# meyer-lab/cmtf-pls

Hardware: AMD Instinct MI355X
Metric: nipals_iters_per_sec (higher is better)
Workload: dtype f32

## Files before the change

### cmtf_pls_amd/_lib.py

```python
from __future__ import annotations

import ctypes
import os
from ctypes import c_char_p, c_double, c_int, c_int64, c_size_t, c_uint64, c_void_p

_HERE = os.path.dirname(os.path.abspath(__file__))
LIB_PATH = os.environ.get("CMTFPLS_LIB") or os.path.join(_HERE, "lib", "libcmtfpls.so")

_P = c_void_p

class XcovBlock(ctypes.Structure):
    _fields_ = [("S", _P), ("S2", _P), ("colcnt", _P), ("n_samples", c_double), ("order", c_int), ("A", c_int), ("B", c_int),
                ("n_squarings", c_int), ("Z", _P), ("wA", _P), ("wB", _P), ("info", _P)]


class KfoldState(ctypes.Structure):
    _fields_ = [("I", c_int), ("A", c_int), ("B", c_int), ("M", c_int), ("K", c_int), ("R", c_int)] + [
        (name, _P) for name in ("fold_of", "S", "mean", "Yk", "Gy", "WA", "WB", "Q", "Wa", "Wb", "T", "Gt", "coef", "Rm", "tm",
                                "Tout", "vec", "n_iter", "status", "part")]


SIGNATURES = {
    "cmtfpls_xcov_iterate_blocks_f64": (c_int, [ctypes.POINTER(XcovBlock), c_int, c_int, _P, _P, _P, _P, _P, c_int, _P, c_size_t, _P]),
    "cmtfpls_abi_version": (c_int, []),
    "cmtfpls_last_error": (c_char_p, []),
    "cmtfpls_clear_error": (c_int, []),
    "cmtfpls_status_to_host": (c_int, [_P, _P, c_size_t, _P, _P]),
    "cmtfpls_colstats_workspace_bytes": (c_size_t, [c_int64, c_int64]),
    "cmtfpls_colstats_f32": (c_int, [_P, c_int64, c_int64, _P, _P, _P, c_size_t, _P]),
    "cmtfpls_colstats_f64": (c_int, [_P, c_int64, c_int64, _P, _P, _P, c_size_t, _P]),
    "cmtfpls_sweep_partials": (c_int, []),
    "cmtfpls_center_f32": (c_int, [_P, c_int64, c_int64, _P, _P, _P, _P]),
    "cmtfpls_center_f64": (c_int, [_P, c_int64, c_int64, _P, _P, _P, _P]),
    "cmtfpls_mode0_contract_workspace_bytes": (c_size_t, [c_int64, c_int64]),
    "cmtfpls_mode0_contract_f32": (c_int, [_P, c_int64, c_int64, _P, _P, c_int, _P, c_size_t, _P]),
    "cmtfpls_mode0_contract_f64": (c_int, [_P, c_int64, c_int64, _P, _P, c_int, _P, c_size_t, _P]),
    "cmtfpls_mode0_contract_yq_f32": (c_int, [_P, c_int64, c_int64, _P, c_int, c_int, _P, _P, c_int, _P, c_size_t, _P]),
    "cmtfpls_mode0_contract_yq_f64": (c_int, [_P, c_int64, c_int64, _P, c_int, c_int, _P, _P, c_int, _P, c_size_t, _P]),
    "cmtfpls_colscale_f64": (c_int, [_P, c_int64, _P, c_double, _P]),
    "cmtfpls_rank1_workspace_bytes": (c_size_t, [c_int, c_int]),
    "cmtfpls_rank1_score_f64": (c_int, [_P, c_int, c_int, _P, _P, _P, c_int, _P, c_int, _P, _P, c_size_t, _P]),
    "cmtfpls_rank1_f64": (c_int, [_P, c_int, c_int, _P, _P, _P, _P, c_int, _P, c_size_t, _P]),
    "cmtfpls_rank1_launches_f64": (c_int, [_P, c_int, c_int, _P, _P, _P, _P, c_int, _P, c_size_t, _P]),
    "cmtfpls_rank1_chain_enable": (None, [c_int]),
    "cmtfpls_rank1_chain_enabled": (c_int, []),
    "cmtfpls_normalize_f64": (c_int, [_P, c_int64, _P, _P]),
    "cmtfpls_rank1_tensor_workspace_bytes": (c_size_t, [_P, c_int]),
    "cmtfpls_rank1_tensor_f64": (c_int, [_P, _P, c_int, c_double, _P, c_int, _P, c_int, _P, c_size_t, _P]),
    "cmtfpls_kron_f64": (c_int, [_P, c_int, _P, c_int, _P, _P]),
    "cmtfpls_xcov_workspace_bytes": (c_size_t, [c_int64, c_int64, c_int]),
    "cmtfpls_xcov_f32": (c_int, [_P, c_int64, c_int64, _P, c_int, c_int, _P, c_int, _P, c_size_t, _P]),
    "cmtfpls_xcov_f64": (c_int, [_P, c_int64, c_int64, _P, c_int, c_int, _P, c_int, _P, c_size_t, _P]),
    "cmtfpls_quadform_f64": (c_int, [_P, c_int, _P, _P, _P, _P]),
    "cmtfpls_xcov_iterate_f64": (c_int, [_P, c_int, c_int, c_int, _P, _P, _P, _P, _P, c_int, _P, _P, _P, c_int, _P, c_size_t, _P, c_size_t, _P]),
    "cmtfpls_s_downdate_f64": (c_int, [_P, c_int, c_int, c_int, _P, _P, _P, _P, _P, _P]),
    "cmtfpls_project_rows_f32": (c_int, [_P, c_int64, c_int, c_int, c_int, _P, _P, _P, _P, c_int, _P]),
    "cmtfpls_project_rows_f64": (c_int, [_P, c_int64, c_int, c_int, c_int, _P, _P, _P, _P, c_int, _P]),
    "cmtfpls_project_rows2_f32": (c_int, [_P, c_int, c_int, _P, _P, _P, _P, c_int, c_int, _P, _P, _P, c_int64, c_int, _P, c_int, _P]),
    "cmtfpls_project_rows2_f64": (c_int, [_P, c_int, c_int, _P, _P, _P, _P, c_int, c_int, _P, _P, _P, c_int64, c_int, _P, c_int, _P]),
    "cmtfpls_project_rows_idx_f32": (c_int, [_P, _P, c_int64, c_int, c_int, c_int, _P, _P, _P, _P, c_int, _P]),
    "cmtfpls_project_rows_idx_f64": (c_int, [_P, _P, c_int64, c_int, c_int, c_int, _P, _P, _P, _P, c_int, _P]),
    "cmtfpls_project_rows2_idx_f32": (c_int, [_P, c_int, c_int, _P, _P, _P, _P, c_int, c_int, _P, _P, _P, _P, c_int64, c_int, _P, c_int, _P]),
    "cmtfpls_project_rows2_idx_f64": (c_int, [_P, c_int, c_int, _P, _P, _P, _P, c_int, c_int, _P, _P, _P, _P, c_int64, c_int, _P, c_int, _P]),
    "cmtfpls_allreduce_sum_f64": (c_int, [_P, _P, c_size_t, _P]),
    "cmtfpls_allreduce_sum_f32": (c_int, [_P, _P, c_size_t, _P]),
    "cmtfpls_axpy_scalar_f64": (c_int, [_P, c_int64, _P, _P, _P]),
    "cmtfpls_xcov_deflate_f32": (c_int, [_P, c_int64, c_int, c_int, _P, c_int, c_int, _P, _P, _P, _P, _P, _P, c_size_t, _P]),
    "cmtfpls_xcov_deflate_f64": (c_int, [_P, c_int64, c_int, c_int, _P, c_int, c_int, _P, _P, _P, _P, _P, _P, c_size_t, _P]),
    "cmtfpls_xcov_stats_workspace_bytes": (c_size_t, [c_int64, c_int64, c_int]),
    "cmtfpls_xcov_stats_f32": (c_int, [_P, c_int64, c_int64, _P, c_int, c_int, _P, _P, _P, c_size_t, _P]),
    "cmtfpls_xcov_stats_f64": (c_int, [_P, c_int64, c_int64, _P, c_int, c_int, _P, _P, _P, c_size_t, _P]),
    "cmtfpls_xcov_ssq_workspace_bytes": (c_size_t, [c_int64, c_int64, c_int]),
    "cmtfpls_xcov_ssq_f32": (c_int, [_P, c_int64, c_int64, _P, c_int, c_int, _P, _P, _P, _P, c_size_t, _P]),
    "cmtfpls_xcov_ssq_f64": (c_int, [_P, c_int64, c_int64, _P, c_int, c_int, _P, _P, _P, _P, c_size_t, _P]),
    "cmtfpls_score_contract_workspace_bytes": (c_size_t, [c_int64, c_int64]),
    "cmtfpls_score_contract_f32": (c_int, [_P, c_int64, c_int, c_int, _P, _P, _P, _P, _P, c_double, _P, _P, _P, _P, c_size_t, _P]),
    "cmtfpls_score_contract_f64": (c_int, [_P, c_int64, c_int, c_int, _P, _P, _P, _P, _P, c_double, _P, _P, _P, _P, c_size_t, _P]),
    "cmtfpls_kr_axpy_f64": (c_int, [_P, c_int, c_int, _P, _P, c_int, c_int, _P, _P]),
    "cmtfpls_xcov_f32_mixed": (c_int, [_P, c_int64, c_int64, _P, c_int, c_int, _P, c_int, _P, c_size_t, _P]),
    "cmtfpls_mttkrp_f32_mixed": (c_int, [_P, c_int64, c_int, c_int, _P, _P, c_int, _P, c_int, _P]),
    "cmtfpls_mttkrp_f32": (c_int, [_P, c_int64, c_int, c_int, _P, _P, c_int, _P, c_int, _P]),
    "cmtfpls_mttkrp_f64": (c_int, [_P, c_int64, c_int, c_int, _P, _P, c_int, _P, c_int, _P]),
    "cmtfpls_score_f32": (c_int, [_P, c_int64, c_int, c_int, _P, _P, _P, _P, _P]),
    "cmtfpls_score_f64": (c_int, [_P, c_int64, c_int, c_int, _P, _P, _P, _P, _P]),
    "cmtfpls_score_s_f64": (c_int, [_P, c_int, c_int, c_int, _P, _P, _P, _P]),
    "cmtfpls_deflate_contract_workspace_bytes": (c_size_t, [c_int64, c_int64]),
    "cmtfpls_deflate_contract_yq_f32": (c_int, [_P, c_int64, c_int, c_int, _P, _P, _P, _P, c_int, c_int, _P, _P, c_int, _P, _P, c_size_t, _P]),
    "cmtfpls_deflate_contract_yq_f64": (c_int, [_P, c_int64, c_int, c_int, _P, _P, _P, _P, c_int, c_int, _P, _P, c_int, _P, _P, c_size_t, _P]),
    "cmtfpls_score_gram_f32": (c_int, [_P, c_int64, c_int, c_int, _P, _P, _P, _P, _P, c_int, c_int, _P, _P]),
    "cmtfpls_score_gram_f64": (c_int, [_P, c_int64, c_int, c_int, _P, _P, _P, _P, _P, c_int, c_int, _P, _P]),
    "cmtfpls_q_update_f64": (c_int, [_P, c_int, c_int, _P, c_int, _P, _P, _P, _P]),
    "cmtfpls_deflate_f32": (c_int, [_P, c_int64, c_int, c_int, _P, _P, _P, _P, _P]),
    "cmtfpls_deflate_f64": (c_int, [_P, c_int64, c_int, c_int, _P, _P, _P, _P, _P]),
    "cmtfpls_score_deflate_f32": (c_int, [_P, c_int64, c_int, c_int, _P, _P, _P, _P, _P, _P]),
    "cmtfpls_score_deflate_f64": (c_int, [_P, c_int64, c_int, c_int, _P, _P, _P, _P, _P, _P]),
    "cmtfpls_small_workspace_bytes": (c_size_t, []),
    "cmtfpls_gram_tn_f64": (c_int, [_P, c_int, c_int, _P, c_int, c_int, c_int64, _P, _P, c_size_t, _P]),
    "cmtfpls_rowdot_f64": (c_int, [_P, c_int, c_int, c_int64, _P, _P, _P, _P, _P, c_size_t, _P]),
    "cmtfpls_scores_mean_f64": (c_int, [_P, c_int, c_int64, _P, _P]),
    "cmtfpls_y_deflate_f64": (c_int, [_P, c_int, c_int, c_int64, _P, c_int, c_int, _P, _P, _P, _P, c_size_t, _P]),
    "cmtfpls_sum_f64": (c_int, [_P, c_int64, _P, _P]),
    "cmtfpls_normal_solve_f64": (c_int, [_P, _P, c_int, _P, c_int, _P]),
    "cmtfpls_normal_solve_workspace_bytes": (c_size_t, [c_int]),
    "cmtfpls_normal_solve_ws_f64": (c_int, [_P, _P, c_int, _P, c_int, _P, c_size_t, _P]),
    "cmtfpls_unit_upper_solve_rows_f64": (c_int, [_P, c_int64, c_int, c_int, _P, _P, _P, _P]),
    "cmtfpls_kr_gram_row_f64": (c_int, [_P, c_int, c_int, c_int, _P, c_int, _P]),
    "cmtfpls_kr_gram_f64": (c_int, [_P, c_int, c_int, _P, c_int, c_double, _P]),
    "cmtfpls_khatri_rao_f64": (c_int, [_P, c_int, _P, c_int, c_int, _P, _P]),
    "cmtfpls_predict_rows_f64": (c_int, [_P, c_int64, c_int, c_int, _P, c_int, _P, _P, c_int, _P]),
    "cmtfpls_recon_f32": (c_int, [_P, c_int64, c_int, c_int, _P, _P, c_int, c_int, _P, _P, _P]),
    "cmtfpls_recon_f64": (c_int, [_P, c_int64, c_int, c_int, _P, _P, c_int, c_int, _P, _P, _P]),
    "cmtfpls_recon_r2_workspace_bytes": (c_size_t, [c_int64, c_int64]),
    "cmtfpls_recon_r2_f32": (c_int, [_P, _P, c_int64, c_int, c_int, _P, _P, c_int, c_int, _P, _P, _P, c_size_t, _P]),
    "cmtfpls_recon_r2_f64": (c_int, [_P, _P, c_int64, c_int, c_int, _P, _P, c_int, c_int, _P, _P, _P, c_size_t, _P]),
    "cmtfpls_loo_fold_workspace_bytes": (c_size_t, [c_int, c_int, c_int, c_int, c_int]),
    "cmtfpls_loo_tpls_f64": (c_int, [_P, _P, _P, _P, c_int, c_int, c_int, c_int, c_int, c_double, c_int, c_int, c_int, _P, _P, _P, c_size_t, _P]),
    "cmtfpls_loo_xcov_fold_workspace_bytes": (c_size_t, [c_int, c_int, c_int, c_int, c_int]),
    "cmtfpls_kfold_xcov_workspace_bytes": (c_size_t, [c_int64, c_int64, c_int, c_int]),
    "cmtfpls_kfold_xcov_f32": (c_int, [_P, c_int64, c_int, c_int, _P, c_int, _P, _P, c_int, _P, _P, _P, _P, _P, c_size_t, _P]),
    "cmtfpls_kfold_xcov_f64": (c_int, [_P, c_int64, c_int, c_int, _P, c_int, _P, _P, c_int, _P, _P, _P, _P, _P, c_size_t, _P]),
    "cmtfpls_kfold_row_tiles": (c_int, [c_int64]),
    "cmtfpls_kfold_part_stride": (c_int, []),
    "cmtfpls_kfold_inner_workspace_bytes": (c_size_t, [c_int, c_int, c_int]),
    "cmtfpls_kfold_inner_f64": (c_int, [ctypes.POINTER(KfoldState), c_int, c_double, c_int, _P, c_size_t, _P]),
    "cmtfpls_kfold_epilogue_f64": (c_int, [ctypes.POINTER(KfoldState), c_int, c_int, _P, _P]),
    "cmtfpls_kfold_inner_coupled_workspace_bytes": (c_size_t, [ctypes.POINTER(KfoldState), c_int]),
    "cmtfpls_kfold_inner_coupled_f64": (c_int, [ctypes.POINTER(KfoldState), c_int, c_int, c_double, c_int, _P, c_size_t, _P]),
    "cmtfpls_kfold_combine_scores_f64": (c_int, [_P, c_int, c_int64, _P, _P]),
    "cmtfpls_kfold_wide_xcov_workspace_bytes": (c_size_t, [c_int64, c_int64, c_int, c_int]),
    "cmtfpls_kfold_wide_xcov_f32": (c_int, [_P, c_int64, c_int, c_int, _P, c_int, _P, _P, c_int, _P, _P, _P, _P, _P, c_size_t, _P]),
    "cmtfpls_kfold_wide_xcov_f64": (c_int, [_P, c_int64, c_int, c_int, _P, c_int, _P, _P, c_int, _P, _P, _P, _P, _P, c_size_t, _P]),
    "cmtfpls_kfold_inner_grouped_f64": (c_int, [ctypes.POINTER(KfoldState), _P, c_int, c_int, c_double, c_int, _P, c_size_t, _P]),
    "cmtfpls_kfold_epilogue_grouped_f64": (c_int, [ctypes.POINTER(KfoldState), _P, c_int, c_int, c_int, _P, _P]),
    "cmtfpls_kfold_epilogue_splits_f64": (c_int, [ctypes.POINTER(KfoldState), c_int, c_int, c_int, _P, _P]),
    "cmtfpls_loo_xcov_f64": (c_int, [_P, _P, _P, _P, c_int, c_int, c_int, c_int, c_int, c_double, c_int, c_int, c_int, _P, _P, _P, c_size_t, _P]),
    "cmtfpls_fit_small_workspace_bytes": (c_size_t, [c_int, c_int, c_int, c_int]),
    "cmtfpls_fit_small_f64": (c_int, [_P, _P, c_int, c_int, c_int, c_int, c_int, c_double, c_int] + [_P] * 11 + [_P, c_size_t, _P]),
    "cmtfpls_add_noise_f32": (c_int, [_P, c_int64, c_double, c_uint64, c_uint64, c_double, _P]),
    "cmtfpls_add_noise_f64": (c_int, [_P, c_int64, c_double, c_uint64, c_uint64, c_double, _P]),
    "cmtfpls_ceiling_max_blocks": (c_int, []),
    "cmtfpls_ceiling_read": (c_int, [_P, c_size_t, c_int64, c_int, _P, c_int, _P]),
    "cmtfpls_ceiling_rmw": (c_int, [_P, c_size_t, c_int64, c_int, c_int, _P]),
    "cmtfpls_ceiling_copy": (c_int, [_P, _P, c_size_t, c_int64, c_int, c_int, _P]),
}

_lib = None


class CmtfplsError(RuntimeError):
    pass


def load():
    global _lib
    if _lib is not None:
        return _lib
    if not os.path.exists(LIB_PATH):
        raise CmtfplsError(
            f"{LIB_PATH} not found: build the HIP extension first (python -c 'import __graft_entry__ as g; g.build()'). "
            "cmtf_pls_amd has no CPU fallback."
        )
    lib = ctypes.CDLL(LIB_PATH)
    for name, (res, args) in SIGNATURES.items():
        fn = getattr(lib, name)
        fn.restype = res
        fn.argtypes = args
    _lib = lib
    return lib


def check(rc: int, what: str = "") -> None:
    if rc != 0:
        msg = load().cmtfpls_last_error()
        raise CmtfplsError(f"{what or 'cmtfpls call'} failed with status {rc}: {msg.decode() if msg else ''}")
```

### cmtf_pls_amd/backend.py

```python
from __future__ import annotations

import ctypes
from typing import Optional, Tuple

import torch

from . import _lib

_SUFFIX = {torch.float32: "f32", torch.float64: "f64"}


def _ptr(t: Optional[torch.Tensor]):
    return None if t is None else t.data_ptr()


class HipBackend:
    name = "hip"

    def __init__(self, device: Optional[torch.device] = None):
        self.lib = _lib.load()
        if not torch.cuda.is_available():
            raise _lib.CmtfplsError("cmtf_pls_amd needs a ROCm GPU (torch.cuda.is_available() is False); there is no CPU fallback")
        self.device = torch.device(device) if device is not None else torch.device("cuda", torch.cuda.current_device())
        self.n_partials = int(self.lib.cmtfpls_sweep_partials())
        self._ws = {}
        self._status_slots = {}
        self.rank1_squarings = 30
        self.rank1_chain_side = 256 if self.lib.cmtfpls_rank1_chain_enabled() else 0

    def _stream(self):
        return torch.cuda.current_stream(self.device).cuda_stream

    def _workspace(self, key: str, nbytes: int) -> torch.Tensor:
        buf = self._ws.get(key)
        if buf is None or buf.numel() < nbytes:
            buf = torch.empty(max(int(nbytes), 256), dtype=torch.uint8, device=self.device)
            self._ws[key] = buf
        return buf

    def clear_error(self) -> bool:
        return bool(self.lib.cmtfpls_clear_error())

    def empty(self, *shape, dtype=torch.float64) -> torch.Tensor:
        return torch.empty(*shape, dtype=dtype, device=self.device)

    def zeros(self, *shape, dtype=torch.float64) -> torch.Tensor:
        return torch.zeros(*shape, dtype=dtype, device=self.device)

    def _fn(self, base: str, X: torch.Tensor):
        if X.dtype not in _SUFFIX:
            raise TypeError(f"X must be float32 or float64 on device, got {X.dtype}")
        assert X.is_contiguous() and X.device == self.device
        return getattr(self.lib, f"cmtfpls_{base}_{_SUFFIX[X.dtype]}")

    def _close_partials(self, part: torch.Tensor) -> torch.Tensor:
        out = self.empty(1)
        _lib.check(self.lib.cmtfpls_sum_f64(_ptr(part), part.numel(), _ptr(out), self._stream()), "sum")
        return out

    def ceiling(self, op: str, buf: torch.Tensor, row_bytes: int = 0, blocks: int = 2048,
                dst: Optional[torch.Tensor] = None, map: int = 0) -> bool:
        nbytes = buf.numel() * buf.element_size()
        if op == "read":
            sink = self._workspace("ceiling_sink", 4 * self.lib.cmtfpls_ceiling_max_blocks())
            rc = self.lib.cmtfpls_ceiling_read(_ptr(buf), nbytes, int(row_bytes), int(map), _ptr(sink), int(blocks), self._stream())
        elif op == "rmw":
            rc = self.lib.cmtfpls_ceiling_rmw(_ptr(buf), nbytes, int(row_bytes), int(map), int(blocks), self._stream())
        elif op == "copy":
            assert dst is not None and dst.numel() * dst.element_size() >= nbytes
            rc = self.lib.cmtfpls_ceiling_copy(_ptr(buf), _ptr(dst), nbytes, int(row_bytes), int(map), int(blocks), self._stream())
        else:
            raise ValueError(op)
        if rc == 4:
            return False
        _lib.check(rc, "ceiling_" + op)
        return True

    def colstats(self, X2: torch.Tensor) -> Tuple[torch.Tensor, torch.Tensor]:
        I, P = X2.shape
        ws = self._workspace("contract", self.lib.cmtfpls_colstats_workspace_bytes(I, P))
        colsum, colcnt = self.empty(P), self.empty(P)
        _lib.check(self._fn("colstats", X2)(_ptr(X2), I, P, _ptr(colsum), _ptr(colcnt), _ptr(ws), ws.numel(), self._stream()), "colstats")
        return colsum, colcnt

    def center(self, X2: torch.Tensor, mean: torch.Tensor, want_rowcnt: bool) -> Tuple[Optional[torch.Tensor], torch.Tensor]:
        I, P = X2.shape
        rowcnt = self.empty(I) if want_rowcnt else None
        part = self.empty(self.n_partials)
        _lib.check(self._fn("center", X2)(_ptr(X2), I, P, _ptr(mean), _ptr(rowcnt), _ptr(part), self._stream()), "center")
        return rowcnt, self._close_partials(part)

    def mode0_contract(self, X2: torch.Tensor, u: torch.Tensor, masked: bool, out: Optional[torch.Tensor] = None) -> torch.Tensor:
        I, P = X2.shape
        ws = self._workspace("contract", self.lib.cmtfpls_mode0_contract_workspace_bytes(I, P))
        Z = out if out is not None else self.empty(P)
        _lib.check(self._fn("mode0_contract", X2)(_ptr(X2), I, P, _ptr(u), _ptr(Z), int(masked), _ptr(ws), ws.numel(), self._stream()), "mode0_contract")
        return Z

    def mode0_contract_yq(self, X2: torch.Tensor, Y: torch.Tensor, q: torch.Tensor, masked: bool,
                          out: torch.Tensor) -> Optional[torch.Tensor]:
        I, P = X2.shape
        ws = self._workspace("contract", self.lib.cmtfpls_mode0_contract_workspace_bytes(I, P))
        rc = self._fn("mode0_contract_yq", X2)(_ptr(X2), I, P, _ptr(Y), Y.stride(0), Y.shape[1], _ptr(q), _ptr(out), int(masked),
                                               _ptr(ws), ws.numel(), self._stream())
        if rc == 4:
            return None
        _lib.check(rc, "mode0_contract_yq")
        return out

    def colscale(self, Z: torch.Tensor, colcnt: torch.Tensor, n_samples: float) -> None:
        _lib.check(self.lib.cmtfpls_colscale_f64(_ptr(Z), Z.numel(), _ptr(colcnt), float(n_samples), self._stream()), "colscale")

    def rank1(self, Z: torch.Tensor, A: int, B: int, wA: torch.Tensor, wB: torch.Tensor,
              info: Optional[torch.Tensor] = None, n_squarings: Optional[int] = None, launches: bool = False) -> None:
        ws = self._workspace("rank1", self.lib.cmtfpls_rank1_workspace_bytes(A, B))
        fn = self.lib.cmtfpls_rank1_launches_f64 if launches else self.lib.cmtfpls_rank1_f64
        _lib.check(fn(_ptr(Z), A, B, _ptr(wA), _ptr(wB), None, _ptr(info), int(n_squarings or self.rank1_squarings),
                      _ptr(ws), ws.numel(), self._stream()), "rank1")

    def rank1_chain_gave_up(self) -> None:
        self.lib.cmtfpls_rank1_chain_enable(0)
        self.rank1_chain_side = 0

    def rank1_tensor(self, Z: torch.Tensor, dims, tol: float, factors: torch.Tensor,
                     info: Optional[torch.Tensor] = None, n_squarings: Optional[int] = None) -> None:
        import ctypes
        arr = (ctypes.c_int * len(dims))(*[int(d) for d in dims])
        ws = self._workspace("rank1t", self.lib.cmtfpls_rank1_tensor_workspace_bytes(arr, len(dims)))
        _lib.check(self.lib.cmtfpls_rank1_tensor_f64(_ptr(Z), arr, len(dims), float(tol), _ptr(factors), factors.stride(0), _ptr(info),
                                                     int(n_squarings or self.rank1_squarings), _ptr(ws), ws.numel(), self._stream()),
                   "rank1_tensor")

    def kron(self, a: torch.Tensor, b: torch.Tensor, out: torch.Tensor) -> torch.Tensor:
        _lib.check(self.lib.cmtfpls_kron_f64(_ptr(a), a.numel(), _ptr(b), b.numel(), _ptr(out), self._stream()), "kron")
        return out

    def normalize(self, v: torch.Tensor) -> None:
        _lib.check(self.lib.cmtfpls_normalize_f64(_ptr(v), v.numel(), None, self._stream()), "normalize")

    def xcov(self, X2: torch.Tensor, Y: torch.Tensor, masked: bool, out: Optional[torch.Tensor] = None,
             mixed: bool = False) -> Optional[torch.Tensor]:
        I, P = X2.shape
        M = Y.shape[1]
        ws = self._workspace("contract", self.lib.cmtfpls_xcov_workspace_bytes(I, P, M))
        S = out if out is not None else self.empty(M, P)
        fn = self.lib.cmtfpls_xcov_f32_mixed if (mixed and X2.dtype == torch.float32) else self._fn("xcov", X2)
        _lib.check(fn(_ptr(X2), I, P, _ptr(Y), Y.stride(0), M, _ptr(S), int(masked), _ptr(ws), ws.numel(), self._stream()), "xcov")
        return S

    def xcov_deflate(self, X2: torch.Tensor, A: int, B: int, Y: torch.Tensor, t: torch.Tensor, wA: torch.Tensor, wB: torch.Tensor,
                     out: torch.Tensor) -> Optional[torch.Tensor]:
        I, P = X2.shape
        M = Y.shape[1]
        if M > 64 or P % 4 != 0 or P != A * B:
            return None
        ws = self._workspace("contract", self.lib.cmtfpls_xcov_ssq_workspace_bytes(I, P, M))
        ssq = self.empty(1)
        rc = self._fn("xcov_deflate", X2)(_ptr(X2), I, A, B, _ptr(Y), Y.stride(0), M, _ptr(t), _ptr(wA), _ptr(wB), _ptr(out), _ptr(ssq),
                                          _ptr(ws), ws.numel(), self._stream())
        if rc == 4:
            return None
        _lib.check(rc, "xcov_deflate")
        return ssq

    def rank1_score(self, Z: torch.Tensor, A: int, B: int, wA: torch.Tensor, wB: torch.Tensor, S: torch.Tensor, tq: torch.Tensor,
                    info: Optional[torch.Tensor] = None, n_squarings: Optional[int] = None) -> torch.Tensor:
        M = S.shape[0]
        assert S.is_contiguous() and S.shape[1] == A * B and tq.numel() >= M
        ws = self._workspace("rank1", self.lib.cmtfpls_rank1_workspace_bytes(A, B))
        _lib.check(self.lib.cmtfpls_rank1_score_f64(_ptr(Z), A, B, _ptr(wA), _ptr(wB), _ptr(info),
                                                    int(n_squarings if n_squarings is not None else self.rank1_squarings),
                                                    _ptr(S), M, _ptr(tq), _ptr(ws), ws.numel(), self._stream()), "rank1_score")
        return tq

    def xcov_ssq(self, X2: torch.Tensor, Y: torch.Tensor, mean: torch.Tensor, out: torch.Tensor):
        I, P = X2.shape
        M = Y.shape[1]
        ws = self._workspace("contract", self.lib.cmtfpls_xcov_ssq_workspace_bytes(I, P, M))
        ssq = self.empty(1)
        assert mean.is_contiguous() and mean.numel() == P and mean.dtype == torch.float64
        _lib.check(self._fn("xcov_ssq", X2)(_ptr(X2), I, P, _ptr(Y), Y.stride(0), M, _ptr(out), _ptr(mean), _ptr(ssq), _ptr(ws), ws.numel(),
                                            self._stream()), "xcov_ssq")
        return out, ssq

    def xcov_stats(self, X2: torch.Tensor, Y: torch.Tensor, out: torch.Tensor):
        I, P = X2.shape
        M = Y.shape[1]
        if M > 64 or not X2.is_contiguous():
            return None
        ws = self._workspace("contract", self.lib.cmtfpls_xcov_stats_workspace_bytes(I, P, M))
        stats = self.empty(2 * P)
        rc = self._fn("xcov_stats", X2)(_ptr(X2), I, P, _ptr(Y), Y.stride(0), M, _ptr(out), _ptr(stats), _ptr(ws), ws.numel(), self._stream())
        if rc == 4:
            return None
        _lib.check(rc, "xcov_stats")
        return out, stats

    def status_snapshot(self, status: torch.Tensor, slot: int, slots: Optional[dict] = None):
        slots = self._status_slots if slots is None else slots
        ent = slots.get((slot, status.numel()))
        if ent is None:
            host, ev = torch.empty(status.numel(), dtype=torch.float64, pin_memory=True), torch.cuda.Event()
            ev.record(torch.cuda.current_stream(self.device))
            ent = slots[(slot, status.numel())] = (host, ev, host.numpy(), host.data_ptr(), ev.cuda_event, status.numel() * 8)
        rc = self.lib.cmtfpls_status_to_host(status.data_ptr(), ent[3], ent[5], ent[4], self._stream())
        if rc:
            _lib.check(rc, "status_to_host")
        return ent

    def status_wait(self, token) -> "np.ndarray":
        token[1].synchronize()
        return token[2]

    def xcov_iterate_plan(self, S: torch.Tensor, A: int, B: int, q_cur: torch.Tensor, Z: torch.Tensor, wA: torch.Tensor,
                          wB: torch.Tensor, status: torch.Tensor, q_new: torch.Tensor, G: torch.Tensor):
        M, P = S.shape
        wc = self._workspace("contract", self.lib.cmtfpls_mode0_contract_workspace_bytes(M, P))
        wr = self._workspace("rank1", self.lib.cmtfpls_rank1_workspace_bytes(A, B))
        keep = (S, q_cur, Z, wA, wB, status, q_new, G, wc, wr)
        fn = self.lib.cmtfpls_xcov_iterate_f64
        head = (_ptr(S), M, A, B, _ptr(q_cur), _ptr(Z), _ptr(wA), _ptr(wB), status[1:3].data_ptr())
        tail = (_ptr(wc), wc.numel(), _ptr(wr), wr.numel())
        qn, Gp, du2 = _ptr(q_new), _ptr(G), status[0:1].data_ptr()
        stream = self._stream

        def enqueue(n_squarings: int, first: bool, _keep=keep) -> None:
            rc = fn(*head, n_squarings, qn, Gp, du2, 1 if first else 0, *tail, stream())
            if rc:
                _lib.check(rc, "xcov_iterate")
        return enqueue

    def xcov_iterate(self, S: torch.Tensor, A: int, B: int, q_cur: torch.Tensor, Z: torch.Tensor, wA: torch.Tensor,
                     wB: torch.Tensor, info: torch.Tensor, n_squarings: int, q_new: torch.Tensor, G: torch.Tensor,
                     du2: torch.Tensor, first: bool) -> None:
        M, P = S.shape
        wc = self._workspace("contract", self.lib.cmtfpls_mode0_contract_workspace_bytes(M, P))
        wr = self._workspace("rank1", self.lib.cmtfpls_rank1_workspace_bytes(A, B))
        _lib.check(self.lib.cmtfpls_xcov_iterate_f64(_ptr(S), M, A, B, _ptr(q_cur), _ptr(Z), _ptr(wA), _ptr(wB), _ptr(info),
                                                     int(n_squarings), _ptr(q_new), _ptr(G), _ptr(du2), int(first),
                                                     _ptr(wc), wc.numel(), _ptr(wr), wr.numel(), self._stream()), "xcov_iterate")

    def xcov_blocks_plan(self, blocks, M: int, q_cur: torch.Tensor, tq: torch.Tensor, q_new: torch.Tensor, G: torch.Tensor,
                         status: torch.Tensor):
        nb = len(blocks)
        if M > 64 or any(b["order"] not in (2, 3) for b in blocks) or tq.numel() != nb * M or not tq.is_contiguous():
            return None
        arr = (_lib.XcovBlock * nb)()
        need = 256
        for i, b in enumerate(blocks):
            for name in ("S", "S2", "colcnt", "Z", "wA", "wB"):
                t = b.get(name)
                assert t is None or (t.is_contiguous() and t.dtype == torch.float64 and t.device == self.device), name
                setattr(arr[i], name, _ptr(t))
            arr[i].n_samples, arr[i].order, arr[i].A, arr[i].B = float(b["n_samples"]), int(b["order"]), int(b["A"]), int(b["B"])
            arr[i].info = status[1 + 2 * i: 3 + 2 * i].data_ptr()
            if b["order"] == 3:
                need = max(need, self.lib.cmtfpls_rank1_workspace_bytes(b["A"], b["B"]))
        wr = self._workspace("rank1", need)
        keep = (blocks, q_cur, tq, q_new, G, status, wr, arr)
        fn, stream = self.lib.cmtfpls_xcov_iterate_blocks_f64, self._stream
        args = (nb, M, _ptr(q_cur), _ptr(tq), _ptr(q_new), _ptr(G), status[0:1].data_ptr())
        tail = (_ptr(wr), wr.numel())

        def enqueue(n_squarings, first: bool, _keep=keep) -> None:
            for i in range(nb):
                arr[i].n_squarings = int(n_squarings[i])
            rc = fn(arr, *args, 1 if first else 0, *tail, stream())
            if rc:
                _lib.check(rc, "xcov_iterate_blocks")
        return enqueue

    def s_downdate(self, S: torch.Tensor, A: int, B: int, ya: torch.Tensor, wA: torch.Tensor, wB: torch.Tensor,
                   q: torch.Tensor, v: torch.Tensor) -> None:
        assert S.is_contiguous() and S.shape[1] == A * B
        _lib.check(self.lib.cmtfpls_s_downdate_f64(_ptr(S), S.shape[0], A, B, _ptr(ya), _ptr(wA), _ptr(wB), _ptr(q), _ptr(v),
                                                   self._stream()), "s_downdate")

    def kr_axpy(self, v: torch.Tensor, A: int, B: int, WA: torch.Tensor, WB: torch.Tensor, k: int, coef: torch.Tensor) -> torch.Tensor:
        assert WA.is_contiguous() and WB.is_contiguous() and WA.shape[1] == WB.shape[1] and coef.numel() >= k
        _lib.check(self.lib.cmtfpls_kr_axpy_f64(_ptr(v), A, B, _ptr(WA), _ptr(WB), WA.shape[1], int(k), _ptr(coef), self._stream()), "kr_axpy")
        return v

    def axpy_scalar(self, y: torch.Tensor, a: torch.Tensor, x: Optional[torch.Tensor] = None) -> torch.Tensor:
        assert y.is_contiguous() and y.dtype == torch.float64 and a.numel() >= 1 and (x is None or (x.is_contiguous() and x.numel() == y.numel()))
        _lib.check(self.lib.cmtfpls_axpy_scalar_f64(_ptr(y), y.numel(), _ptr(a), _ptr(x), self._stream()), "axpy_scalar")
        return y

    def total(self, v: torch.Tensor) -> torch.Tensor:
        assert v.is_contiguous() and v.dtype == torch.float64
        return self._close_partials(v)

    def quadform(self, G: torch.Tensor, q: torch.Tensor, q_old: torch.Tensor, out: torch.Tensor) -> torch.Tensor:
        _lib.check(self.lib.cmtfpls_quadform_f64(_ptr(G), G.shape[0], _ptr(q), _ptr(q_old), _ptr(out), self._stream()), "quadform")
        return out

    def mttkrp(self, X2: torch.Tensor, A: int, B: int, WA: torch.Tensor, WB: torch.Tensor, out: torch.Tensor,
               mixed: bool = False) -> Optional[torch.Tensor]:
        R = WA.shape[1]
        assert WA.is_contiguous() and WB.is_contiguous() and out.stride(1) == 1
        fn = self.lib.cmtfpls_mttkrp_f32_mixed if (mixed and X2.dtype == torch.float32) else self._fn("mttkrp", X2)
        rc = fn(_ptr(X2), X2.shape[0], A, B, _ptr(WA), _ptr(WB), R, _ptr(out), out.stride(0), self._stream())
        if rc == 4:
            return None
        _lib.check(rc, "mttkrp")
        return out

    def score(self, X2, A, B, wA, wB, rowcnt, out) -> torch.Tensor:
        _lib.check(self._fn("score", X2)(_ptr(X2), X2.shape[0], A, B, _ptr(wA), _ptr(wB), _ptr(rowcnt), _ptr(out), self._stream()), "score")
        return out

    def score_s(self, S, A, B, wA, wB, out) -> torch.Tensor:
        assert S.dtype == torch.float64 and S.is_contiguous()
        _lib.check(self.lib.cmtfpls_score_s_f64(_ptr(S), S.shape[0], A, B, _ptr(wA), _ptr(wB), _ptr(out), self._stream()), "score_s")
        return out

    def score_contract(self, X2, A, B, wA, wB, shift, t, Z, sub_own=None, add_other=None, alpha: float = 1.0,
                       csum: Optional[torch.Tensor] = None) -> Optional[torch.Tensor]:
        I, P = X2.shape
        if not X2.is_contiguous() or P != A * B:
            return None
        for v in (sub_own, add_other):
            assert v is None or (v.is_contiguous() and v.numel() == I and v.dtype == torch.float64)
        nbytes = self.lib.cmtfpls_score_contract_workspace_bytes(I, P)
        ws = self._workspace("score_contract", max(nbytes, 256))
        rc = self._fn("score_contract", X2)(_ptr(X2), I, A, B, _ptr(wA), _ptr(wB), _ptr(shift), _ptr(sub_own), _ptr(add_other), float(alpha),
                                            _ptr(t), _ptr(Z), _ptr(csum), _ptr(ws), ws.numel(), self._stream())
        if rc == 4:
            return None
        _lib.check(rc, "score_contract")
        return Z

    def score_gram(self, X2, A, B, wA, wB, rowcnt, out, Y: torch.Tensor, qpart: torch.Tensor) -> Optional[torch.Tensor]:
        assert qpart.numel() >= self.n_partials * Y.shape[1] and qpart.is_contiguous()
        rc = self._fn("score_gram", X2)(_ptr(X2), X2.shape[0], A, B, _ptr(wA), _ptr(wB), _ptr(rowcnt), _ptr(out),
                                        _ptr(Y), Y.stride(0), Y.shape[1], _ptr(qpart), self._stream())
        if rc == 4:
            return None
        _lib.check(rc, "score_gram")
        return out

    def q_update(self, q: torch.Tensor, qpart: Optional[torch.Tensor] = None, normalize: bool = True,
                 G: Optional[torch.Tensor] = None, q_prev: Optional[torch.Tensor] = None,
                 du2: Optional[torch.Tensor] = None, nparts: Optional[int] = None) -> None:
        M = q.numel()
        nrows = (nparts or self.n_partials) if qpart is not None else 0
        assert qpart is None or (qpart.is_contiguous() and qpart.numel() >= nrows * M)
        _lib.check(self.lib.cmtfpls_q_update_f64(_ptr(qpart), nrows, M, _ptr(q), int(normalize),
                                                 _ptr(G), _ptr(q_prev), _ptr(du2), self._stream()), "q_update")

    def deflate(self, X2, A, B, t, wA, wB) -> torch.Tensor:
        part = self.empty(self.n_partials)
        _lib.check(self._fn("deflate", X2)(_ptr(X2), X2.shape[0], A, B, _ptr(t), _ptr(wA), _ptr(wB), _ptr(part), self._stream()), "deflate")
        return self._close_partials(part)

    def deflate_contract_yq(self, X2, A, B, t, wA, wB, Y: torch.Tensor, q: torch.Tensor, masked: bool,
                            out: torch.Tensor) -> Optional[torch.Tensor]:
        I, P = X2.shape
        ws = self._workspace("deflate_contract", self.lib.cmtfpls_deflate_contract_workspace_bytes(I, P))
        ssq = self.empty(1)
        rc = self._fn("deflate_contract_yq", X2)(_ptr(X2), I, A, B, _ptr(t), _ptr(wA), _ptr(wB), _ptr(Y), Y.stride(0), Y.shape[1],
                                                 _ptr(q), _ptr(out), int(masked), _ptr(ssq), _ptr(ws), ws.numel(), self._stream())
        if rc == 4:
            return None
        _lib.check(rc, "deflate_contract_yq")
        return ssq

    def score_deflate(self, X2, A, B, wA, wB, rowcnt, out) -> Optional[torch.Tensor]:
        part = self.empty(self.n_partials)
        rc = self._fn("score_deflate", X2)(_ptr(X2), X2.shape[0], A, B, _ptr(wA), _ptr(wB), _ptr(rowcnt), _ptr(out), _ptr(part), self._stream())
        if rc == 4:
            return None
        _lib.check(rc, "score_deflate")
        return self._close_partials(part)

    def gram_tn(self, A: torch.Tensor, B: torch.Tensor, out: Optional[torch.Tensor] = None) -> torch.Tensor:
        if A.dim() == 1:
            A = A.unsqueeze(1)
        if B.dim() == 1:
            B = B.unsqueeze(1)
        assert A.stride(1) == 1 and B.stride(1) == 1 and A.shape[0] == B.shape[0]
        a, b = A.shape[1], B.shape[1]
        ws = self._workspace("small", self.lib.cmtfpls_small_workspace_bytes())
        C = out if out is not None else self.empty(a, b)
        assert C.numel() == a * b and C.is_contiguous()
        _lib.check(self.lib.cmtfpls_gram_tn_f64(_ptr(A), A.stride(0), a, _ptr(B), B.stride(0), b, A.shape[0], _ptr(C),
                                                _ptr(ws), ws.numel(), self._stream()), "gram_tn")
        return C

    def rowdot(self, Y: torch.Tensor, q: torch.Tensor, u_out: torch.Tensor, u_old: Optional[torch.Tensor],
               du2: Optional[torch.Tensor] = None) -> Optional[torch.Tensor]:
        ws = self._workspace("small", self.lib.cmtfpls_small_workspace_bytes())
        if u_old is not None and du2 is None:
            du2 = self.empty(1)
        _lib.check(self.lib.cmtfpls_rowdot_f64(_ptr(Y), Y.stride(0), Y.shape[1], Y.shape[0], _ptr(q), _ptr(u_out), _ptr(u_old),
                                               _ptr(du2) if u_old is not None else None,
                                               _ptr(ws), ws.numel(), self._stream()), "rowdot")
        return du2 if u_old is not None else None

    def normal_solve(self, G: torch.Tensor, g: torch.Tensor, out: Optional[torch.Tensor] = None) -> torch.Tensor:
        k = G.shape[0]
        assert G.is_contiguous() and G.shape == (k, k) and g.numel() == k
        b = out if out is not None else self.empty(k)
        if k <= 64:
            _lib.check(self.lib.cmtfpls_normal_solve_f64(_ptr(G), _ptr(g), k, _ptr(b), 1, self._stream()), "normal_solve")
        else:
            ws = self._workspace("normal_solve", self.lib.cmtfpls_normal_solve_workspace_bytes(k))
            _lib.check(self.lib.cmtfpls_normal_solve_ws_f64(_ptr(G), _ptr(g), k, _ptr(b), 1, _ptr(ws), ws.numel(), self._stream()),
                       "normal_solve")
        return b

    def unit_upper_solve_rows(self, M: torch.Tensor, U: torch.Tensor, shift: Optional[torch.Tensor] = None,
                              nan_flag: Optional[torch.Tensor] = None) -> torch.Tensor:
        I, R = M.shape
        assert M.stride(1) == 1 and U.is_contiguous() and U.shape == (R, R)
        assert shift is None or (shift.is_contiguous() and shift.numel() == R and shift.dtype == torch.float64)
        assert nan_flag is None or nan_flag.dtype == torch.int32
        _lib.check(self.lib.cmtfpls_unit_upper_solve_rows_f64(_ptr(M), I, M.stride(0), R, _ptr(U), _ptr(shift), _ptr(nan_flag),
                                                              self._stream()), "unit_upper_solve_rows")
        return M

    def kr_gram_row(self, L: torch.Tensor, a: int, g: torch.Tensor, first: bool) -> torch.Tensor:
        assert L.is_contiguous() and g.is_contiguous() and g.numel() >= a
        _lib.check(self.lib.cmtfpls_kr_gram_row_f64(_ptr(L), L.shape[0], L.shape[1], int(a), _ptr(g), int(first), self._stream()), "kr_gram_row")
        return g

    def kr_gram(self, L: torch.Tensor, G: torch.Tensor, first: bool) -> torch.Tensor:
        n, R = L.shape
        assert L.is_contiguous() and G.is_contiguous() and G.numel() == R * R
        _lib.check(self.lib.cmtfpls_kr_gram_f64(_ptr(L), n, R, _ptr(G), int(first), 1.0, self._stream()), "kr_gram")
        return G

    def khatri_rao(self, Am: torch.Tensor, Bm: torch.Tensor) -> torch.Tensor:
        na, R = Am.shape
        nb = Bm.shape[0]
        assert Am.is_contiguous() and Bm.is_contiguous() and Bm.shape[1] == R
        out = self.empty(na * nb, R)
        _lib.check(self.lib.cmtfpls_khatri_rao_f64(_ptr(Am), na, _ptr(Bm), nb, R, _ptr(out), self._stream()), "khatri_rao")
        return out

    def project_rows(self, X2: torch.Tensor, A: int, B: int, WA: torch.Tensor, WB: torch.Tensor, mean: Optional[torch.Tensor],
                     out: torch.Tensor, rows: Optional[torch.Tensor] = None) -> Optional[torch.Tensor]:
        I, R = X2.shape[0], WA.shape[1]
        assert WA.is_contiguous() and WB.is_contiguous() and out.stride(1) == 1 and out.shape == (I, R)
        if rows is not None:
            assert rows.dtype == torch.int64 and rows.is_contiguous() and rows.device == self.device
            rc = self._fn("project_rows_idx", X2)(_ptr(X2), _ptr(rows), rows.numel(), A, B, R, _ptr(WA), _ptr(WB), _ptr(mean), _ptr(out),
                                                  out.stride(0), self._stream())
        else:
            rc = self._fn("project_rows", X2)(_ptr(X2), I, A, B, R, _ptr(WA), _ptr(WB), _ptr(mean), _ptr(out), out.stride(0), self._stream())
        if rc == 4:
            return None
        _lib.check(rc, "project_rows")
        return out

    def project_rows2(self, X2s, As, Bs, WAs, WBs, means, out: torch.Tensor, rows: Optional[torch.Tensor] = None) -> Optional[torch.Tensor]:
        I, R = X2s[0].shape[0], WAs[0].shape[1]
        if X2s[0].dtype != X2s[1].dtype or X2s[1].shape[0] != I:
            return None
        assert all(w.is_contiguous() for w in list(WAs) + list(WBs)) and out.stride(1) == 1 and out.shape == (I, R)
        head = (_ptr(X2s[0]), As[0], Bs[0], _ptr(WAs[0]), _ptr(WBs[0]), _ptr(means[0]),
                _ptr(X2s[1]), As[1], Bs[1], _ptr(WAs[1]), _ptr(WBs[1]), _ptr(means[1]))
        if rows is not None:
            assert rows.dtype == torch.int64 and rows.is_contiguous() and rows.device == self.device
            rc = self._fn("project_rows2_idx", X2s[0])(*head, _ptr(rows), rows.numel(), R, _ptr(out), out.stride(0), self._stream())
        else:
            rc = self._fn("project_rows2", X2s[0])(*head, I, R, _ptr(out), out.stride(0), self._stream())
        if rc == 4:
            return None
        _lib.check(rc, "project_rows2")
        return out

    def predict_rows(self, S: torch.Tensor, Bm: torch.Tensor, mean: Optional[torch.Tensor]) -> Optional[torch.Tensor]:
        I, R = S.shape
        M = Bm.shape[1]
        assert S.stride(1) == 1 and Bm.is_contiguous() and Bm.shape[0] == R
        out = self.empty(I, M)
        rc = self.lib.cmtfpls_predict_rows_f64(_ptr(S), I, S.stride(0), R, _ptr(Bm), M, _ptr(mean), _ptr(out), M, self._stream())
        if rc == 4:
            return None
        _lib.check(rc, "predict_rows")
        return out

    def recon(self, T: torch.Tensor, WA: torch.Tensor, WB: torch.Tensor, mean: Optional[torch.Tensor], out: torch.Tensor) -> Optional[torch.Tensor]:
        I, R = T.shape
        A, B = WA.shape[0], WB.shape[0]
        assert T.stride(1) == 1 and WA.is_contiguous() and WB.is_contiguous() and out.is_contiguous() and out.numel() == I * A * B
        rc = self._fn("recon", out)(_ptr(T), I, T.stride(0), R, _ptr(WA), _ptr(WB), A, B, _ptr(mean), _ptr(out), self._stream())
        if rc == 4:
            return None
        _lib.check(rc, "recon")
        return out

    def recon_r2(self, X2: torch.Tensor, T: torch.Tensor, WA: torch.Tensor, WB: torch.Tensor, mean: Optional[torch.Tensor]) -> Optional[torch.Tensor]:
        I, P = X2.shape
        R = T.shape[1]
        A, B = WA.shape[0], WB.shape[0]
        assert X2.is_contiguous() and T.stride(1) == 1 and WA.is_contiguous() and WB.is_contiguous() and P == A * B
        ws = self._workspace("recon_r2", self.lib.cmtfpls_recon_r2_workspace_bytes(I, P))
        out = self.empty(2)
        rc = self._fn("recon_r2", X2)(_ptr(X2), _ptr(T), I, T.stride(0), R, _ptr(WA), _ptr(WB), A, B, _ptr(mean), _ptr(out),
                                     _ptr(ws), ws.numel(), self._stream())
        if rc == 4:
            return None
        _lib.check(rc, "recon_r2")
        return out

    def loo_tpls(self, X2: torch.Tensor, Y: torch.Tensor, A: int, B: int, R: int, tol: float, max_iter: int,
                 max_ws_bytes: Optional[int] = None, forms=("lds", "xcov")) -> Optional[Tuple[torch.Tensor, torch.Tensor, str]]:
        I, P = X2.shape
        M = Y.shape[1]
        assert X2.dtype == torch.float64 and Y.dtype == torch.float64 and X2.is_contiguous() and Y.is_contiguous() and P == A * B
        colsum_x, _ = self.colstats(X2)
        colsum_y, _ = self.colstats(Y)
        Ypred = self.empty(I, M)
        n_iter = torch.zeros(I, R, dtype=torch.int32, device=self.device)
        for form, per_fn, fn in (("lds", self.lib.cmtfpls_loo_fold_workspace_bytes, self.lib.cmtfpls_loo_tpls_f64),
                                 ("xcov", self.lib.cmtfpls_loo_xcov_fold_workspace_bytes, self.lib.cmtfpls_loo_xcov_f64)):
            if form not in forms:
                continue
            if fn(_ptr(X2), _ptr(Y), _ptr(colsum_x), _ptr(colsum_y), I, A, B, M, R, float(tol), int(max_iter), 0, 1, _ptr(Ypred),
                  _ptr(n_iter), None, 0, self._stream()) == 4:
                continue
            per = per_fn(I, A, B, M, R)
            budget = max_ws_bytes
            if budget is None:
                budget = (4 << 30) if form == "lds" else max(4 << 30, torch.cuda.mem_get_info(self.device)[0] // 3)
            chunk = max(1, min(I, int(budget // max(per, 1))))
            if form == "xcov":
                chunk = min(chunk, 512)
            declined = False
            ws = None
            for f0 in range(0, I, chunk):
                nf = min(chunk, I - f0)
                if ws is None:
                    ws = self._workspace("loo", per * min(chunk, I))
                rc = fn(_ptr(X2), _ptr(Y), _ptr(colsum_x), _ptr(colsum_y), I, A, B, M, R, float(tol), int(max_iter),
                        f0, nf, _ptr(Ypred), _ptr(n_iter), _ptr(ws), ws.numel(), self._stream())
                if rc == 4:
                    declined = True
                    break
                _lib.check(rc, "loo_" + form)
            if not declined:
                return Ypred, n_iter, form
        return None

    def kfold_xcov(self, X2: torch.Tensor, A: int, B: int, Y: torch.Tensor, order: torch.Tensor, fold_off: torch.Tensor, K: int,
                   ydev: torch.Tensor, S: torch.Tensor, mean: torch.Tensor) -> Optional[torch.Tensor]:
        I, P = X2.shape
        M = Y.shape[1]
        assert Y.dtype == torch.float64 and Y.is_contiguous() and order.dtype == torch.int32 and fold_off.dtype == torch.int32 and P == A * B
        ws = torch.empty(max(int(self.lib.cmtfpls_kfold_xcov_workspace_bytes(I, P, M, K)), 256), dtype=torch.uint8, device=self.device)
        stats = self.empty(2 * P)
        rc = self._fn("kfold_xcov", X2)(_ptr(X2), I, A, B, _ptr(Y), M, _ptr(order), _ptr(fold_off), K, _ptr(ydev), _ptr(S), _ptr(mean),
                                        _ptr(stats), _ptr(ws), ws.numel(), self._stream())
        if rc == 4:
            return None
        _lib.check(rc, "kfold_xcov")
        return stats

    def kfold_inner(self, state, a: int, tol: float, max_iter: int, ws: torch.Tensor) -> Optional[bool]:
        rc = self.lib.cmtfpls_kfold_inner_f64(ctypes.byref(state), int(a), float(tol), int(max_iter), _ptr(ws), ws.numel(), self._stream())
        if rc == 4:
            return None
        _lib.check(rc, "kfold_inner")
        return True

    def kfold_inner_workspace_bytes(self, A: int, B: int, K: int) -> int:
        return int(self.lib.cmtfpls_kfold_inner_workspace_bytes(A, B, K))

    def kfold_row_tiles(self, I: int) -> Tuple[int, int]:
        return int(self.lib.cmtfpls_kfold_row_tiles(I)), int(self.lib.cmtfpls_kfold_part_stride())

    def kfold_epilogue(self, state, stage: int, a: int, src: Optional[torch.Tensor]) -> Optional[bool]:
        rc = self.lib.cmtfpls_kfold_epilogue_f64(ctypes.byref(state), int(stage), int(a), _ptr(src), self._stream())
        if rc == 4:
            return None
        _lib.check(rc, "kfold_epilogue")
        return True

    def kfold_inner_coupled(self, views, a: int, tol: float, max_iter: int, ws: torch.Tensor) -> Optional[bool]:
        rc = self.lib.cmtfpls_kfold_inner_coupled_f64(views, len(views), int(a), float(tol), int(max_iter), _ptr(ws), ws.numel(),
                                                      self._stream())
        if rc == 4:
            return None
        _lib.check(rc, "kfold_inner_coupled")
        return True

    def kfold_inner_coupled_workspace_bytes(self, views) -> int:
        return int(self.lib.cmtfpls_kfold_inner_coupled_workspace_bytes(views, len(views)))

    def kfold_combine_scores(self, sc: torch.Tensor, out: torch.Tensor) -> torch.Tensor:
        assert sc.is_contiguous() and out.is_contiguous() and sc[0].numel() == out.numel()
        _lib.check(self.lib.cmtfpls_kfold_combine_scores_f64(_ptr(sc), sc.shape[0], out.numel(), _ptr(out), self._stream()),
                   "kfold_combine_scores")
        return out

    def kfold_wide_xcov(self, X2: torch.Tensor, A: int, B: int, Y: torch.Tensor, order: torch.Tensor, fold_off: torch.Tensor, K: int,
                        ydev: torch.Tensor, S: torch.Tensor, mean: torch.Tensor) -> Optional[torch.Tensor]:
        I, P = X2.shape
        W = Y.shape[1]
        assert Y.dtype == torch.float64 and Y.is_contiguous() and ydev.is_contiguous() and S.is_contiguous() and P == A * B
        assert order.dtype == torch.int32 and fold_off.dtype == torch.int32 and S.numel() == K * W * P and mean.numel() == K * P
        ws = torch.empty(max(int(self.lib.cmtfpls_kfold_wide_xcov_workspace_bytes(I, P, W, K)), 256), dtype=torch.uint8, device=self.device)
        stats = self.empty(2 * P)
        rc = self._fn("kfold_wide_xcov", X2)(_ptr(X2), I, A, B, _ptr(Y), W, _ptr(order), _ptr(fold_off), K, _ptr(ydev), _ptr(S),
                                             _ptr(mean), _ptr(stats), _ptr(ws), ws.numel(), self._stream())
        if rc == 4:
            return None
        _lib.check(rc, "kfold_wide_xcov")
        return stats

    def kfold_inner_grouped(self, state, model_fold: torch.Tensor, groups: int, a: int, tol: float, max_iter: int,
                            ws: torch.Tensor) -> Optional[bool]:
        assert model_fold.dtype == torch.int32 and model_fold.numel() == state.K
        rc = self.lib.cmtfpls_kfold_inner_grouped_f64(ctypes.byref(state), _ptr(model_fold), int(groups), int(a), float(tol), int(max_iter),
                                                      _ptr(ws), ws.numel(), self._stream())
        if rc == 4:
            return None
        _lib.check(rc, "kfold_inner_grouped")
        return True

    def kfold_epilogue_grouped(self, state, model_fold: torch.Tensor, groups: int, stage: int, a: int,
                               src: Optional[torch.Tensor]) -> Optional[bool]:
        assert model_fold.dtype == torch.int32 and model_fold.numel() == state.K
        rc = self.lib.cmtfpls_kfold_epilogue_grouped_f64(ctypes.byref(state), _ptr(model_fold), int(groups), int(stage), int(a), _ptr(src),
                                                         self._stream())
        if rc == 4:
            return None
        _lib.check(rc, "kfold_epilogue_grouped")
        return True

    def kfold_epilogue_splits(self, state, splits: int, stage: int, a: int, src: Optional[torch.Tensor]) -> Optional[bool]:
        rc = self.lib.cmtfpls_kfold_epilogue_splits_f64(ctypes.byref(state), int(splits), int(stage), int(a), _ptr(src), self._stream())
        if rc == 4:
            return None
        _lib.check(rc, "kfold_epilogue_splits")
        return True

    def fit_small(self, X2: torch.Tensor, Y: torch.Tensor, A: int, B: int, R: int, tol: float, max_iter: int):
        I, P = X2.shape
        M = Y.shape[1]
        if X2.dtype != torch.float64 or Y.dtype != torch.float64 or not (X2.is_contiguous() and Y.is_contiguous()) or I >= 2 ** 31 or P != A * B:
            return None
        nbytes = self.lib.cmtfpls_fit_small_workspace_bytes(I, A, B, M)
        T, U = self.empty(I, R), self.empty(I, R)
        WA, WB, Q = self.empty(A, R), self.empty(B, R), self.empty(M, R)
        small = self.empty(R * R + 2 * (R + 1))
        xm, ym = self.empty(P), self.empty(M)
        ints = torch.zeros(R + 1, dtype=torch.int32, device=self.device)
        ws = self._workspace("fit_small", max(nbytes, 256))
        rc = self.lib.cmtfpls_fit_small_f64(_ptr(X2), _ptr(Y), I, A, B, M, R, float(tol), int(max_iter), _ptr(T), _ptr(U), _ptr(WA), _ptr(WB),
                                            _ptr(Q), _ptr(small), small[R * R:].data_ptr(), _ptr(xm), _ptr(ym), _ptr(ints),
                                            ints[R:].data_ptr(), _ptr(ws), ws.numel(), self._stream())
        if rc == 4:
            return None
        _lib.check(rc, "fit_small")
        ih = ints.cpu().numpy()
        if ih[R] != 0:
            return None
        sh = small.cpu().numpy()
        return {"T": T, "U": U, "WA": WA, "WB": WB, "Q": Q, "x_mean": xm, "y_mean": ym, "coef": sh[:R * R].reshape(R, R).copy(),
                "ssq": sh[R * R:].reshape(R + 1, 2).copy(), "n_iter": [int(v) for v in ih[:R]]}

    def add_noise(self, X: torch.Tensor, sigma: float, seed: int, offset: int = 0, nan_fraction: float = 0.0) -> torch.Tensor:
        assert X.is_contiguous() and X.device == self.device
        _lib.check(self._fn("add_noise", X)(_ptr(X), X.numel(), float(sigma), int(seed) & (2 ** 64 - 1), int(offset), float(nan_fraction),
                                            self._stream()), "add_noise")
        return X

    def scores_mean(self, Ts: torch.Tensor, out: torch.Tensor) -> torch.Tensor:
        nb, I = Ts.shape
        _lib.check(self.lib.cmtfpls_scores_mean_f64(_ptr(Ts), nb, I, _ptr(out), self._stream()), "scores_mean")
        return out

    def y_deflate(self, Y: torch.Tensor, T: torch.Tensor, ncols: int, b: torch.Tensor, q: torch.Tensor) -> torch.Tensor:
        ws = self._workspace("small", self.lib.cmtfpls_small_workspace_bytes())
        ssq = self.empty(1)
        _lib.check(self.lib.cmtfpls_y_deflate_f64(_ptr(Y), Y.stride(0), Y.shape[1], Y.shape[0], _ptr(T), T.stride(0), ncols, _ptr(b), _ptr(q),
                                                  _ptr(ssq), _ptr(ws), ws.numel(), self._stream()), "y_deflate")
        return ssq
```

### cmtf_pls_amd/csrc/rank1.hip

```cpp
#include "common.hpp"
#include <atomic>

namespace cmtfpls {

constexpr int kTile = 16;
constexpr int kMaxTiles = 256;
constexpr int kMaxSteps = 48;

struct Rank1Ctl {
  int done;
  int final_buf;
  int steps_used;
  int last_step;
  double pad[6];
};
__host__ __device__ __forceinline__ size_t rank1_ctl_bytes(int nt) {
  return sizeof(Rank1Ctl) + ((size_t)(kMaxSteps + 2) * nt + 2 * (size_t)nt * nt) * sizeof(double);
}
__device__ __forceinline__ double* ctl_trace(Rank1Ctl* c, int nt, int step) { return reinterpret_cast<double*>(c + 1) + (size_t)step * nt; }
__device__ __forceinline__ double* ctl_fro(Rank1Ctl* c, int nt, int which) {
  return reinterpret_cast<double*>(c + 1) + (size_t)(kMaxSteps + 2) * nt + (size_t)which * nt * nt;
}

__device__ __forceinline__ double pow2_scale_from_trace(const double* parts, int nt, double* tr_out) {
  double tr = 0.0;
  for (int i = 0; i < nt; ++i) tr += parts[i];
  *tr_out = tr;
  if (!(tr > 0.0) || !isfinite(tr)) return 1.0;
  int e;
  frexp(tr, &e);
  return ldexp(1.0, -e);
}

typedef double d4r_t __attribute__((ext_vector_type(4)));

__global__ __launch_bounds__(kTile* kTile) void syrk_step_kernel(const double* __restrict__ M, int n, int k, int ld,
                                                                double* __restrict__ C, Rank1Ctl* __restrict__ ctl,
                                                                int step, int out_buf, double* __restrict__ C_keep) {
  __shared__ double red[4][kTile * kTile];
  __shared__ double diag[kTile];
  __shared__ double s_scale;
  __shared__ int s_done;
  __shared__ double fsum[4];
  __shared__ double tr_s[kMaxTiles];
  const int tx = threadIdx.x, ty = threadIdx.y, tid = ty * kTile + tx;
  const int lane = tid & 63, wv = tid >> 6, ri = lane & 15, kq = lane >> 4;
  const int nt = (n + kTile - 1) / kTile;
  const int i0 = blockIdx.y * kTile, j0 = blockIdx.x * kTile;

  constexpr int KC = 128, KW = 8;
  const bool ra = (i0 + ri) < n, rb = (j0 + ri) < n;
  const double* __restrict__ rowa = M + (int64_t)(ra ? i0 + ri : 0) * ld;
  const double* __restrict__ rowb = M + (int64_t)(rb ? j0 + ri : 0) * ld;
  const int cl = 32 * wv + KW * kq;
  double a[KW], b[KW];
#pragma unroll
  for (int s2 = 0; s2 < KW; ++s2) {
    const int c = cl + s2;
    const int cc = (c < k) ? c : 0;
    a[s2] = rowa[cc];
    b[s2] = rowb[cc];
  }

  double fro_in = 0.0;
  if (step >= 1) {
    int zero = 0;
    asm volatile("" : "+v"(zero));
    const int last_in = (&ctl->last_step)[zero];
    const int done_in = (&ctl->done)[zero] | ((last_in >= 0 && last_in < step) ? 1 : 0);
    const double* fp = ctl_fro(ctl, nt, (step - 1) & 1);
    const double trv = ctl_trace(ctl, nt, step - 1)[(tid < nt) ? tid : 0];
    double f = fp[(tid < nt * nt) ? tid : 0];
    if (tid < nt) tr_s[tid] = trv;
    if (tid >= nt * nt) f = 0.0;
    for (int i = tid + kTile * kTile; i < nt * nt; i += kTile * kTile) f += fp[i];
    f = wave_sum(f);
    if ((tid & 63) == 0) fsum[tid >> 6] = f;
    if (tid == 0) s_done = done_in;
    __syncthreads();
    fro_in = ((fsum[0] + fsum[1]) + fsum[2]) + fsum[3];
  }
  if (tid == 0) {
    int done = 0;
    double scale = 1.0;
    if (step == 0) {
      if (blockIdx.x == 0 && blockIdx.y == 0) { ctl->done = 0; ctl->final_buf = -1; ctl->steps_used = 0; ctl->last_step = -1; }
    } else {
      done = s_done;
      if (!done) {
        double tr1;
        scale = pow2_scale_from_trace(tr_s, nt, &tr1);
        const double rho = fro_in / (tr1 * tr1);
        const bool rank_one_in = !(tr1 > 0.0) || rho >= 1.0 - 1e-13;
        const bool rank_one_out = rho >= 1.0 - 1e-7;
        if (blockIdx.x == 0 && blockIdx.y == 0) {
          if (rank_one_in) { ctl->done = 1; ctl->final_buf = out_buf ^ 1; }
          else {
            ctl->steps_used = step;
            if (rank_one_out) { ctl->last_step = step; ctl->final_buf = out_buf; }
          }
        }
        if (rank_one_in) done = 1;
      }
    }
    s_scale = scale;
    s_done = done;
  }
  __syncthreads();
  if (s_done) return;
  const double scale = s_scale;

  d4r_t acc = d4r_t{0.0, 0.0, 0.0, 0.0};
  for (int kk = 0; kk < k; kk += KC) {
    if (kk > 0) {
#pragma unroll
      for (int s2 = 0; s2 < KW; ++s2) {
        const int c = kk + cl + s2;
        const int cc = (c < k) ? c : 0;
        a[s2] = rowa[cc];
        b[s2] = rowb[cc];
      }
    }
#pragma unroll
    for (int s2 = 0; s2 < KW; ++s2) {
      const bool cok = (kk + cl + s2) < k;
      const double av = (ra && cok) ? a[s2] : 0.0;
      const double bv = (rb && cok) ? b[s2] : 0.0;
      acc = __builtin_amdgcn_mfma_f64_16x16x4f64(av, bv, acc, 0, 0, 0);
    }
  }
#pragma unroll
  for (int e = 0; e < 4; ++e) red[wv][(kq + 4 * e) * kTile + ri] = acc[e];
  __syncthreads();
  double cacc = ((red[0][tid] + red[1][tid]) + red[2][tid]) + red[3][tid];
  cacc *= scale * scale;
  const bool inside = (i0 + ty < n && j0 + tx < n);
  if (inside) C[(int64_t)(i0 + ty) * n + (j0 + tx)] = cacc;
  if (inside && C_keep) C_keep[(int64_t)(i0 + ty) * n + (j0 + tx)] = cacc;
  {
    double sq = inside ? cacc * cacc : 0.0;
    sq = wave_sum(sq);
    if ((tid & 63) == 0) fsum[tid >> 6] = sq;
    __syncthreads();
    if (tid == 0) ctl_fro(ctl, nt, step & 1)[blockIdx.y * nt + blockIdx.x] = ((fsum[0] + fsum[1]) + fsum[2]) + fsum[3];
  }
  if (blockIdx.x == blockIdx.y) {
    if (tx == ty) diag[tx] = (i0 + ty < n) ? cacc : 0.0;
    __syncthreads();
    if (tid == 0) {
      double t = 0.0;
      for (int l = 0; l < kTile; ++l) t += diag[l];
      ctl_trace(ctl, nt, step)[blockIdx.x] = t;
    }
  }
}

constexpr unsigned long long kChainEmpty = ~0ull;
constexpr int kChainMaxSteps = 31;
constexpr int kChainSpin = 1 << 15;

__device__ __forceinline__ double chain_ld(const double* p) {
  return __longlong_as_double((long long)__hip_atomic_load(reinterpret_cast<const unsigned long long*>(p), __ATOMIC_RELAXED, __HIP_MEMORY_SCOPE_AGENT));
}
__device__ __forceinline__ void chain_st(double* p, double v) {
  unsigned long long b = (unsigned long long)__double_as_longlong(v);
  if (b == kChainEmpty) b = 0x7FF8000000000000ull;
  __hip_atomic_store(reinterpret_cast<unsigned long long*>(p), b, __ATOMIC_RELAXED, __HIP_MEMORY_SCOPE_AGENT);
}
__device__ __forceinline__ bool chain_empty(double v) { return (unsigned long long)__double_as_longlong(v) == kChainEmpty; }

__global__ __launch_bounds__(256) void chain_preset_kernel(unsigned long long* __restrict__ p, int64_t n) {
  for (int64_t i = (int64_t)blockIdx.x * 256 + threadIdx.x; i < n; i += (int64_t)gridDim.x * 256) p[i] = kChainEmpty;
}

#ifdef CMTFPLS_CHAIN_PROFILE
__device__ unsigned long long g_chain_prof[1024];
#define CHAIN_STAMP(slot) do { if (first_wg && tid == 0 && step < 32) g_chain_prof[step * 8 + (slot)] = __builtin_amdgcn_s_memrealtime(); } while (0)
#define CHAIN_COUNT(slot, v) do { if (first_wg && tid == 0 && step < 32) g_chain_prof[step * 8 + (slot)] = (unsigned long long)(v); } while (0)
#else
#define CHAIN_STAMP(slot) do { } while (0)
#define CHAIN_COUNT(slot, v) do { } while (0)
#endif

__global__ __launch_bounds__(kTile* kTile) void syrk_chain_kernel(const double* __restrict__ M0, int n, int k0,
                                                                 double* gbufs, double* trs, double* fros, double* gave_up,
                                                                 Rank1Ctl* __restrict__ ctl, int n_squarings) {
  constexpr int KC = 128, KW = 8, LDP = KC + 2;
  __shared__ __attribute__((aligned(16))) double pan[2][kTile][LDP];
  __shared__ double red[2][4][kTile * kTile];
  __shared__ double diag[2][kTile];
  __shared__ double fsum[2][4];
  __shared__ double cfro[2][4];
  __shared__ double ctr[2][kTile];
  __shared__ int cdead[2];
  const int tx = threadIdx.x, ty = threadIdx.y, tid = ty * kTile + tx;
  const int lane = tid & 63, wv = tid >> 6, ri = lane & 15, kq = lane >> 4;
  const int nt = (n + kTile - 1) / kTile, nt2 = nt * nt;
  const int i0 = blockIdx.y * kTile, j0 = blockIdx.x * kTile;
  const bool first_wg = blockIdx.x == 0 && blockIdx.y == 0;
  const bool ra = (i0 + ri) < n, rb = (j0 + ri) < n;
  const int cl = 32 * wv + KW * kq;
  const int64_t nn = (int64_t)n * n;
  const double qnan = __longlong_as_double(0x7FF8000000000000ll);
  bool dead = false;
  if (first_wg && tid == 0) { ctl->done = 0; ctl->final_buf = -1; ctl->steps_used = 0; ctl->last_step = -1; }
  if (tid < 2) cdead[tid] = 0;
  int last_step = -1;
  for (int step = 0; step <= n_squarings; ++step) {
    if (last_step >= 0) break;
    const int par = step & 1;
    const double* __restrict__ M = step == 0 ? M0 : gbufs + (int64_t)(step - 1) * nn;
    const int k = step == 0 ? k0 : n, ld = k;
    double* C = gbufs + (int64_t)step * nn;
    double a[KW], b[KW];
    double scale = 1.0;
    bool input_is_result = false;
    d4r_t acc = d4r_t{0.0, 0.0, 0.0, 0.0};
    CHAIN_STAMP(0);
    for (int kk = 0; kk < k; kk += KC) {
      if (step == 0) {
        const double* __restrict__ rowa = M + (int64_t)(ra ? i0 + ri : 0) * ld;
        const double* __restrict__ rowb = M + (int64_t)(rb ? j0 + ri : 0) * ld;
#pragma unroll
        for (int s2 = 0; s2 < KW; ++s2) {
          const int c = kk + cl + s2;
          const int cc = (c < k) ? c : 0;
          a[s2] = rowa[cc];
          b[s2] = rowb[cc];
        }
      } else {
        double va[8], vb[8], trv = 0.0, f = 0.0;
        const bool first_chunk = kk == 0;
        const double* tp = trs + (int64_t)(step - 1) * nt;
        const double* fp = fros + (int64_t)(step - 1) * nt2;
        unsigned offa[8], offb[8];
#pragma unroll
        for (int i = 0; i < 8; ++i) {
          const int e = tid + 256 * i, r = e >> 7, c = kk + (e & 127);
          const int cc = (c < k) ? c : 0;
          const int rra = (i0 + r < n) ? i0 + r : 0, rrb = (j0 + r < n) ? j0 + r : 0;
          offa[i] = (unsigned)(rra * ld + cc);
          offb[i] = (unsigned)(rrb * ld + cc);
        }
        int spins = 0;
        for (;;) {
          bool ok = true;
#pragma unroll
          for (int i = 0; i < 8; ++i) {
            va[i] = chain_ld(M + offa[i]);
            vb[i] = chain_ld(M + offb[i]);
          }
          if (first_chunk) {
            f = chain_ld(fp + ((tid < nt2) ? tid : 0));
            ok = !chain_empty(f);
            if (wv == 0) {
              trv = chain_ld(tp + ((lane < nt) ? lane : 0));
              ok = ok && !chain_empty(trv);
            }
          }
#pragma unroll
          for (int i = 0; i < 8; ++i) ok = ok && !chain_empty(va[i]) && !chain_empty(vb[i]);
          if (dead || __all(ok)) break;
          if (++spins > kChainSpin) {
            dead = true;
            if (lane == 0) chain_st(gave_up, 1.0);
            break;
          }
        }
        CHAIN_STAMP(1);
        CHAIN_COUNT(7, spins);
        if (kk > 0) __syncthreads();
#pragma unroll
        for (int i = 0; i < 8; ++i) {
          const int e = tid + 256 * i, r = e >> 7, c = e & 127;
          pan[0][r][c] = dead ? qnan : va[i];
          pan[1][r][c] = dead ? qnan : vb[i];
        }
        if (first_chunk) {
          const double fw = wave_sum((tid < nt2) ? f : 0.0);
          if (lane == 0) cfro[par][wv] = fw;
          if (wv == 0 && lane < nt) ctr[par][lane] = trv;
          if (dead && lane == 0) cdead[par] = 1;
        }
        __syncthreads();
        CHAIN_STAMP(2);
        if (first_chunk) {
          const double fro_in = ((cfro[par][0] + cfro[par][1]) + cfro[par][2]) + cfro[par][3];
          double tr1 = 0.0;
          for (int i = 0; i < nt; ++i) tr1 += ctr[par][i];
          if ((tr1 > 0.0) && isfinite(tr1)) {
            int e;
            frexp(tr1, &e);
            scale = ldexp(1.0, -e);
          }
          const bool gone = cdead[par] != 0;
          const double rho = fro_in / (tr1 * tr1);
          const bool rank_one_in = !gone && (!(tr1 > 0.0) || rho >= 1.0 - 1e-13);
          const bool rank_one_out = !gone && rho >= 1.0 - 1e-7;
          if (first_wg && tid == 0) {
            if (rank_one_in) { ctl->done = 1; ctl->final_buf = step - 1; }
            else {
              ctl->steps_used = step;
              if (rank_one_out) { ctl->last_step = step; ctl->final_buf = step; }
            }
          }
          if (rank_one_in) { input_is_result = true; break; }
          if (rank_one_out) last_step = step;
        }
#pragma unroll
        for (int s2 = 0; s2 < KW; ++s2) {
          a[s2] = pan[0][ri][cl + s2];
          b[s2] = pan[1][ri][cl + s2];
        }
      }
#pragma unroll
      for (int s2 = 0; s2 < KW; ++s2) {
        const bool cok = (kk + cl + s2) < k;
        const double av = (ra && cok) ? a[s2] : 0.0;
        const double bv = (rb && cok) ? b[s2] : 0.0;
        acc = __builtin_amdgcn_mfma_f64_16x16x4f64(av, bv, acc, 0, 0, 0);
      }
    }
    if (input_is_result) break;
    CHAIN_STAMP(3);
#pragma unroll
    for (int e = 0; e < 4; ++e) red[par][wv][(kq + 4 * e) * kTile + ri] = acc[e];
    __syncthreads();
    CHAIN_STAMP(4);
    double cacc = ((red[par][0][tid] + red[par][1][tid]) + red[par][2][tid]) + red[par][3][tid];
    cacc *= scale * scale;
    const bool inside = (i0 + ty < n && j0 + tx < n);
    if (inside) chain_st(C + (int64_t)(i0 + ty) * n + (j0 + tx), cacc);
    CHAIN_STAMP(5);
    double sq = inside ? cacc * cacc : 0.0;
    sq = wave_sum(sq);
    if ((tid & 63) == 0) fsum[par][tid >> 6] = sq;
    if (blockIdx.x == blockIdx.y && tx == ty) diag[par][tx] = (i0 + ty < n) ? cacc : 0.0;
    __syncthreads();
    if (tid == 0) {
      chain_st(fros + (int64_t)step * nt2 + blockIdx.y * nt + blockIdx.x, ((fsum[par][0] + fsum[par][1]) + fsum[par][2]) + fsum[par][3]);
      if (blockIdx.x == blockIdx.y) {
        double t = 0.0;
        for (int l = 0; l < kTile; ++l) t += diag[par][l];
        chain_st(trs + (int64_t)step * nt + blockIdx.x, t);
      }
    }
    CHAIN_STAMP(6);
  }
}

__global__ __launch_bounds__(256) void transpose_kernel(const double* __restrict__ Z, int A, int B, double* __restrict__ Zt) {
  const int64_t idx = (int64_t)blockIdx.x * 256 + threadIdx.x;
  if (idx >= (int64_t)A * B) return;
  const int b = (int)(idx / A), a = (int)(idx % A);
  Zt[idx] = Z[(int64_t)a * B + b];
}

__global__ __launch_bounds__(256) void rank1_seed_xy_kernel(const double* __restrict__ M, int n, int k,
                                                           const double* __restrict__ gbase, int64_t gstride,
                                                           const double* __restrict__ G0,
                                                           const Rank1Ctl* __restrict__ ctl, int last_buf, int ny_blocks,
                                                           double* __restrict__ y, double* __restrict__ x) {
  extern __shared__ double seed[];
  __shared__ double red[16];
  __shared__ double rsum[8][33];
  __shared__ double bestv[4];
  __shared__ int besti[4];
  const int fb = (ctl->final_buf >= 0) ? ctl->final_buf : last_buf;
  const double* G = gbase + (int64_t)fb * gstride;
  double bv = -1.0;
  int bi = 0;
  for (int i = threadIdx.x; i < n; i += 256) {
    const double d = G[(int64_t)i * n + i];
    if (d > bv) { bv = d; bi = i; }
  }
#pragma unroll
  for (int m = 32; m > 0; m >>= 1) {
    const double ov = __shfl_xor(bv, m, 64);
    const int oi = __shfl_xor(bi, m, 64);
    if (ov > bv || (ov == bv && oi < bi)) { bv = ov; bi = oi; }
  }
  if ((threadIdx.x & 63) == 0) { bestv[threadIdx.x >> 6] = bv; besti[threadIdx.x >> 6] = bi; }
  __syncthreads();
  bv = bestv[0];
  bi = besti[0];
  for (int w = 1; w < 4; ++w)
    if (bestv[w] > bv || (bestv[w] == bv && besti[w] < bi)) { bv = bestv[w]; bi = besti[w]; }
  double ss = 0.0;
  for (int i = threadIdx.x; i < n; i += 256) {
    const double g = G[(int64_t)bi * n + i];
    seed[i] = g;
    ss = fma(g, g, ss);
  }
  const double nrm = sqrt(block_sum(ss, red));
  for (int i = threadIdx.x; i < n; i += 256) seed[i] = seed[i] / nrm;
  __syncthreads();
  if ((int)blockIdx.x >= ny_blocks) {
    const int j = ((int)blockIdx.x - ny_blocks) * 4 + (threadIdx.x >> 6);
    const int lane = threadIdx.x & 63;
    if (j < n) {
      double s = 0.0;
      for (int i = lane; i < n; i += 64) s = fma(G0[(int64_t)j * n + i], seed[i], s);
      s = wave_sum(s);
      if (lane == 0) x[j] = s;
    }
    return;
  }
  const int cx = threadIdx.x & 31, ry = threadIdx.x >> 5;
  const int c = blockIdx.x * 32 + cx;
  double s = 0.0;
  if (c < k)
    for (int j = ry; j < n; j += 8) s = fma(M[(int64_t)j * k + c], seed[j], s);
  rsum[ry][cx] = s;
  __syncthreads();
  if (ry == 0 && c < k) {
    double tot = 0.0;
#pragma unroll
    for (int g = 0; g < 8; ++g) tot += rsum[g][cx];
    y[c] = tot;
  }
}

__device__ __forceinline__ void rank1_write_info(double* __restrict__ info, const Rank1Ctl* __restrict__ ctl, const double* gave) {
  if (!info) return;
  if (gave && !chain_empty(chain_ld(gave))) { info[0] = 0.0; info[1] = -1.0; return; }
  info[0] = (ctl->done || ctl->last_step >= 0) ? 1.0 : 0.0;
  info[1] = (double)ctl->steps_used;
}

__device__ __forceinline__ void rank1_final_body(const double* x, const double* y,
                                                 int n, int k, int x_is_A, const Rank1Ctl* __restrict__ ctl,
                                                 double* __restrict__ wA, double* __restrict__ wB,
                                                 double* __restrict__ sigma, double* __restrict__ info, const double* gave) {
  __shared__ double red[2][16];
  __shared__ double bestv[16];
  __shared__ int besti[16];
  double sx = 0.0, sy = 0.0;
  for (int i = threadIdx.x; i < n; i += 1024) sx = fma(x[i], x[i], sx);
  for (int i = threadIdx.x; i < k; i += 1024) sy = fma(y[i], y[i], sy);
  const double nx = sqrt(block_sum(sx, red[0]));
  const double ny = sqrt(block_sum(sy, red[1]));
  const double* vb = x_is_A ? y : x;
  const int nb = x_is_A ? k : n;
  double bv = -1.0;
  int bi = 0;
  for (int i = threadIdx.x; i < nb; i += 1024) {
    const double d = fabs(vb[i]);
    if (d > bv) { bv = d; bi = i; }
  }
#pragma unroll
  for (int m = 32; m > 0; m >>= 1) {
    const double ov = __shfl_xor(bv, m, 64);
    const int oi = __shfl_xor(bi, m, 64);
    if (ov > bv || (ov == bv && oi < bi)) { bv = ov; bi = oi; }
  }
  if ((threadIdx.x & 63) == 0) { bestv[threadIdx.x >> 6] = bv; besti[threadIdx.x >> 6] = bi; }
  __syncthreads();
  bv = bestv[0];
  bi = besti[0];
  for (int w = 1; w < 16; ++w)
    if (bestv[w] > bv || (bestv[w] == bv && besti[w] < bi)) { bv = bestv[w]; bi = besti[w]; }
  const bool gv = gave && !chain_empty(chain_ld(gave));
  const double sgn = gv ? __longlong_as_double(0x7FF8000000000000ll) : ((vb[bi] < 0.0) ? -1.0 : 1.0);
  double* ox = x_is_A ? wA : wB;
  double* oy = x_is_A ? wB : wA;
  for (int i = threadIdx.x; i < n; i += 1024) ox[i] = sgn * (x[i] / nx);
  for (int i = threadIdx.x; i < k; i += 1024) oy[i] = sgn * (y[i] / ny);
  if (threadIdx.x == 0) {
    if (sigma) sigma[0] = nx / ny;
    rank1_write_info(info, ctl, gave);
  }
}

__global__ __launch_bounds__(1024) void rank1_final_kernel(const double* __restrict__ x, const double* __restrict__ y,
                                                          int n, int k, int x_is_A, const Rank1Ctl* __restrict__ ctl,
                                                          double* __restrict__ wA, double* __restrict__ wB,
                                                          double* __restrict__ sigma, double* __restrict__ info, const double* gave) {
  rank1_final_body(x, y, n, k, x_is_A, ctl, wA, wB, sigma, info, gave);
}

__global__ __launch_bounds__(1024) void rank1_final_score_kernel(const double* __restrict__ x, const double* __restrict__ y,
                                                                int n, int k, int x_is_A, const Rank1Ctl* __restrict__ ctl,
                                                                double* __restrict__ wA, double* __restrict__ wB,
                                                                double* __restrict__ info, const double* __restrict__ S, int A, int B,
                                                                double* __restrict__ t, const double* gave) {
  extern __shared__ double lds[];
  __shared__ double red[2][16];
  __shared__ double bestv[16];
  __shared__ int besti[16];
  double* sA = lds;
  double* sB = lds + ((A + 1) & ~1);
  double sx = 0.0, sy = 0.0;
  for (int i = threadIdx.x; i < n; i += 1024) sx = fma(x[i], x[i], sx);
  for (int i = threadIdx.x; i < k; i += 1024) sy = fma(y[i], y[i], sy);
  const double nx = sqrt(block_sum(sx, red[0]));
  const double ny = sqrt(block_sum(sy, red[1]));
  const double* vb = x_is_A ? y : x;
  const int nb = x_is_A ? k : n;
  double bv = -1.0;
  int bi = 0;
  for (int i = threadIdx.x; i < nb; i += 1024) {
    const double d = fabs(vb[i]);
    if (d > bv) { bv = d; bi = i; }
  }
#pragma unroll
  for (int m = 32; m > 0; m >>= 1) {
    const double ov = __shfl_xor(bv, m, 64);
    const int oi = __shfl_xor(bi, m, 64);
    if (ov > bv || (ov == bv && oi < bi)) { bv = ov; bi = oi; }
  }
  if ((threadIdx.x & 63) == 0) { bestv[threadIdx.x >> 6] = bv; besti[threadIdx.x >> 6] = bi; }
  __syncthreads();
  bv = bestv[0];
  bi = besti[0];
  for (int w = 1; w < 16; ++w)
    if (bestv[w] > bv || (bestv[w] == bv && besti[w] < bi)) { bv = bestv[w]; bi = besti[w]; }
  const bool gv = gave && !chain_empty(chain_ld(gave));
  const double sgn = gv ? __longlong_as_double(0x7FF8000000000000ll) : ((vb[bi] < 0.0) ? -1.0 : 1.0);
  double* lx = x_is_A ? sA : sB;
  double* ly = x_is_A ? sB : sA;
  double* ox = x_is_A ? wA : wB;
  double* oy = x_is_A ? wB : wA;
  const bool store = blockIdx.x == 0;
  for (int i = threadIdx.x; i < n; i += 1024) {
    const double v = sgn * (x[i] / nx);
    lx[i] = v;
    if (store) ox[i] = v;
  }
  for (int i = threadIdx.x; i < k; i += 1024) {
    const double v = sgn * (y[i] / ny);
    ly[i] = v;
    if (store) oy[i] = v;
  }
  if (store && threadIdx.x == 0) rank1_write_info(info, ctl, gave);
  __syncthreads();
  using VT = Pack<double, 2>;
  const int64_t P = (int64_t)A * B;
  const int64_t step = (int64_t)1024 * 2;
  const double* __restrict__ xr = S + (int64_t)blockIdx.x * P;
  KronWalk w((int64_t)threadIdx.x * 2, step, B);
  double acc = 0.0;
  int64_t c = (int64_t)threadIdx.x * 2;
  constexpr int UN = 4;
  for (; c + (UN - 1) * step < P; c += UN * step) {
    VT xs[UN];
#pragma unroll
    for (int u = 0; u < UN; ++u) xs[u] = ld_stream(reinterpret_cast<const VT*>(xr + c + u * step));
#pragma unroll
    for (int u = 0; u < UN; ++u) {
      double d = 0.0;
      d = fma(xs[u].e[0], sB[w.k], d);
      d = fma(xs[u].e[1], sB[w.k + 1], d);
      acc = fma(sA[w.j], d, acc);
      w.next();
    }
  }
  for (; c < P; c += step) {
    const VT xv = ld_stream(reinterpret_cast<const VT*>(xr + c));
    double d = 0.0;
    d = fma(xv.e[0], sB[w.k], d);
    d = fma(xv.e[1], sB[w.k + 1], d);
    acc = fma(sA[w.j], d, acc);
    w.next();
  }
  acc = block_sum(acc, red[0]);
  if (threadIdx.x == 0) t[blockIdx.x] = acc;
}

static inline size_t align_up(size_t x, size_t a) { return (x + a - 1) / a * a; }

static std::atomic<int> g_chain_on{1};

static int chain_slots() {
  static int slots = 0;
  if (slots == 0) {
    int dev = 0, cus = 0;
    if (hipGetDevice(&dev) != hipSuccess || hipDeviceGetAttribute(&cus, hipDeviceAttributeMultiprocessorCount, dev) != hipSuccess || cus <= 0) cus = 256;
    slots = 2 * cus;
  }
  return slots;
}

}

using namespace cmtfpls;

extern "C" {

size_t cmtfpls_rank1_workspace_bytes(int A, int B) {
  if (A <= 0 || B <= 0) return 0;
  const size_t n = (size_t)(A < B ? A : B), k = (size_t)(A < B ? B : A);
  const size_t nt = (n + kTile - 1) / kTile;
  const size_t chain = nt * nt <= 256 ? align_up(((size_t)(kChainMaxSteps + 1) * (n * n + nt + nt * nt) + 1) * sizeof(double), 256) : 0;
  return align_up(rank1_ctl_bytes((int)nt), 256) + 3 * align_up(n * n * sizeof(double), 256) +
         align_up((size_t)A * B * sizeof(double), 256) + align_up(n * sizeof(double), 256) + align_up(k * sizeof(double), 256) + chain;
}

static int rank1_run(const double* Z, int A, int B, double* wA, double* wB, double* sigma, double* info,
                     int n_squarings, void* ws, size_t ws_bytes, void* stream, const double* S, int M, double* tq, bool allow_chain = true);

int cmtfpls_rank1_f64(const double* Z, int A, int B, double* wA, double* wB, double* sigma, double* info,
                      int n_squarings, void* ws, size_t ws_bytes, void* stream) {
  return rank1_run(Z, A, B, wA, wB, sigma, info, n_squarings, ws, ws_bytes, stream, nullptr, 0, nullptr);
}

#ifdef CMTFPLS_CHAIN_PROFILE
int cmtfpls_debug_chain_prof(unsigned long long* out) { return (int)hipMemcpyFromSymbol(out, HIP_SYMBOL(g_chain_prof), sizeof(unsigned long long) * 1024); }
#endif
void cmtfpls_rank1_chain_enable(int on) { g_chain_on.store((on == 1 || on == 2) ? on : 0, std::memory_order_relaxed); }
int cmtfpls_rank1_chain_enabled(void) { return g_chain_on.load(std::memory_order_relaxed); }

int cmtfpls_rank1_launches_f64(const double* Z, int A, int B, double* wA, double* wB, double* sigma, double* info,
                               int n_squarings, void* ws, size_t ws_bytes, void* stream) {
  return rank1_run(Z, A, B, wA, wB, sigma, info, n_squarings, ws, ws_bytes, stream, nullptr, 0, nullptr, false);
}

int cmtfpls_rank1_score_f64(const double* Z, int A, int B, double* wA, double* wB, double* info, int n_squarings,
                            const double* S, int M, double* tq, void* ws, size_t ws_bytes, void* stream) {
  if (!S || !tq || M <= 0) { set_error("rank1_score: bad argument"); return CMTFPLS_EINVAL; }
  const int64_t P = (int64_t)A * B;
  if (M > 64 || P < 8192 || (B % 2) != 0 || ((size_t)(((A + 1) & ~1) + B) * sizeof(double)) > 60 * 1024 ||
      (reinterpret_cast<uintptr_t>(S) & 15) != 0) {
    int rc = cmtfpls_rank1_f64(Z, A, B, wA, wB, nullptr, info, n_squarings, ws, ws_bytes, stream);
    if (rc == CMTFPLS_OK) rc = cmtfpls_score_s_f64(S, M, A, B, wA, wB, tq, stream);
    return rc;
  }
  return rank1_run(Z, A, B, wA, wB, nullptr, info, n_squarings, ws, ws_bytes, stream, S, M, tq);
}

static int rank1_run(const double* Z, int A, int B, double* wA, double* wB, double* sigma, double* info,
                     int n_squarings, void* ws, size_t ws_bytes, void* stream, const double* S, int M, double* tq, bool allow_chain) {
  if (!Z || !wA || !wB || A <= 0 || B <= 0) { set_error("rank1: bad argument"); return CMTFPLS_EINVAL; }
  const int n = A < B ? A : B, k = A < B ? B : A;
  if (n > kTile * kMaxTiles) { set_error("rank1: min(A, B) > 4096 unsupported"); return CMTFPLS_EUNSUPPORTED; }
  if ((size_t)n * sizeof(double) > 64 * 1024) { set_error("rank1: seed exceeds the LDS"); return CMTFPLS_EUNSUPPORTED; }
  if (n_squarings < 1) n_squarings = 1;
  if (n_squarings > kMaxSteps) n_squarings = kMaxSteps;
  if (!ws || ws_bytes < cmtfpls_rank1_workspace_bytes(A, B)) { set_error("rank1: workspace too small"); return CMTFPLS_EWORKSPACE; }
  hipStream_t st = (hipStream_t)stream;
  char* p = static_cast<char*>(ws);
  Rank1Ctl* ctl = reinterpret_cast<Rank1Ctl*>(p);
  p += align_up(rank1_ctl_bytes((n + kTile - 1) / kTile), 256);
  double* buf0 = reinterpret_cast<double*>(p);
  p += align_up((size_t)n * n * sizeof(double), 256);
  double* buf1 = reinterpret_cast<double*>(p);
  p += align_up((size_t)n * n * sizeof(double), 256);
  double* g0keep = reinterpret_cast<double*>(p);
  p += align_up((size_t)n * n * sizeof(double), 256);
  double* Zt = reinterpret_cast<double*>(p);
  p += align_up((size_t)A * B * sizeof(double), 256);
  double* xv = reinterpret_cast<double*>(p);
  p += align_up((size_t)n * sizeof(double), 256);
  double* yv = reinterpret_cast<double*>(p);
  p += align_up((size_t)k * sizeof(double), 256);
  double* chain_region = reinterpret_cast<double*>(p);

  const double* M0 = Z;
  if (A > B) {
    const int64_t tot = (int64_t)A * B;
    hipLaunchKernelGGL(transpose_kernel, dim3((unsigned)((tot + 255) / 256)), dim3(256), 0, st, Z, A, B, Zt);
    M0 = Zt;
  }
  const int nt = (n + kTile - 1) / kTile;
  const dim3 grid(nt, nt), block(kTile, kTile);
  const int ny_blocks = (k + 31) / 32;
  const double* gave = nullptr;
  if (allow_chain && g_chain_on.load(std::memory_order_relaxed) && nt * nt <= 256 && nt * nt <= chain_slots() && n_squarings <= kChainMaxSteps) {
    const size_t nn = (size_t)n * n, steps = (size_t)n_squarings + 1;
    double* gbufs = chain_region;
    double* trs = gbufs + steps * nn;
    double* fros = trs + steps * nt;
    double* gave_up = fros + steps * (size_t)nt * nt;
    gave = gave_up;
    const int64_t words = (int64_t)(steps * (nn + nt + (size_t)nt * nt) + 1);
    hipLaunchKernelGGL(chain_preset_kernel, dim3((unsigned)((words + 2047) / 2048)), dim3(256), 0, st, reinterpret_cast<unsigned long long*>(chain_region), words);
    const dim3 cgrid(nt, (g_chain_on.load(std::memory_order_relaxed) == 2 && nt > 1) ? nt - 1 : nt);
    hipLaunchKernelGGL(syrk_chain_kernel, cgrid, block, 0, st, M0, n, k, gbufs, trs, fros, gave_up, ctl, n_squarings);
    hipLaunchKernelGGL(rank1_seed_xy_kernel, dim3(ny_blocks + (n + 3) / 4), dim3(256), (size_t)n * sizeof(double), st,
                       M0, n, k, gbufs, (int64_t)nn, gbufs, ctl, n_squarings, ny_blocks, yv, xv);
  } else {
    hipLaunchKernelGGL(syrk_step_kernel, grid, block, 0, st, M0, n, k, k, buf0, ctl, 0, 0, g0keep);
    for (int s = 1; s <= n_squarings; ++s) {
      const double* in = (s & 1) ? buf0 : buf1;
      double* out = (s & 1) ? buf1 : buf0;
      hipLaunchKernelGGL(syrk_step_kernel, grid, block, 0, st, in, n, n, n, out, ctl, s, s & 1, (double*)nullptr);
    }
    hipLaunchKernelGGL(rank1_seed_xy_kernel, dim3(ny_blocks + (n + 3) / 4), dim3(256), (size_t)n * sizeof(double), st,
                       M0, n, k, buf0, (int64_t)(buf1 - buf0), g0keep, ctl, n_squarings & 1, ny_blocks, yv, xv);
  }
  if (S) {
    const size_t lds = (size_t)(((A + 1) & ~1) + B) * sizeof(double);
    hipLaunchKernelGGL(rank1_final_score_kernel, dim3((unsigned)M), dim3(1024), lds, st, xv, yv, n, k, (A <= B) ? 1 : 0, ctl, wA, wB, info,
                       S, A, B, tq, gave);
    return check_launch("rank1_score");
  }
  hipLaunchKernelGGL(rank1_final_kernel, dim3(1), dim3(1024), 0, st, xv, yv, n, k, (A <= B) ? 1 : 0, ctl, wA, wB, sigma, info, gave);
  return check_launch("rank1");
}

}
```

### cmtf_pls_amd/engine.py

```python
from __future__ import annotations

import contextlib
import math
from typing import Dict, List, Optional

import torch

from .fitrun import FitRun
from .options import EngineOptions, default_options, set_default_options
from .projection import ProjectionMixin
from .state import (MAX_COMPONENTS, MAX_ORDER, MAX_RANK1_SIDE, MAX_TENSOR_MODE, BlockState, FitState, split_trailing,
                    validate_limits)


class Comm:

    def __init__(self, group=None, enabled: Optional[bool] = None, force: bool = False):
        import torch.distributed as dist

        self._dist = dist
        self.group = group
        on = dist.is_available() and dist.is_initialized() if enabled is None else enabled
        self.world = dist.get_world_size(group) if on else 1
        self.rank = dist.get_rank(group) if on else 0
        self.sharded = self.world > 1 or (bool(force) and on)
        self.n_collectives = 0
        self.backend = str(dist.get_backend(group)) if on else None
        self.capturable = self.backend == "nccl"

    def allreduce(self, t: torch.Tensor) -> torch.Tensor:
        if self.sharded:
            self._dist.all_reduce(t, op=self._dist.ReduceOp.SUM, group=self.group)
            self.n_collectives += 1
        return t


class _NoComm:
    world, rank, sharded = 1, 0, False

    def allreduce(self, t):
        return t


class NipalsEngine(ProjectionMixin):
    def __init__(self, backend, comm=None, options: Optional[EngineOptions] = None):
        self.be = backend
        self.comm = comm if comm is not None else _NoComm()
        self.opt = options if options is not None else default_options()
        self.last_projection: Dict[str, object] = {}

    def device_ctx(self):
        dev = getattr(self.be, "device", None)
        if isinstance(dev, torch.device) and dev.type == "cuda":
            return torch.cuda.device(dev)
        return contextlib.nullcontext()

    def _prepare_block(self, X: torch.Tensor, n_total: int, defer_centring: bool = False) -> BlockState:
        be, comm = self.be, self.comm
        I = X.shape[0]
        X2 = X.view(I, -1)
        P = X2.shape[1]
        A, B = split_trailing(X.shape)
        colsum, colcnt = be.colstats(X2)
        comm.allreduce(colsum)
        comm.allreduce(colcnt)
        mean = colsum / colcnt
        has_miss = bool((colcnt.sum() < float(n_total) * P - 0.5).item())
        blk = BlockState(shape=tuple(X.shape), A=A, B=B, mean=mean, has_miss=has_miss,
                         colcnt=colcnt if has_miss else None, rowcnt=None, ssq0=float("nan"), dtype=X.dtype)
        if not defer_centring:
            self._centre_block(blk, X)
        return blk

    def _centre_block(self, blk: BlockState, X: torch.Tensor) -> None:
        rowcnt, ssq0 = self.be.center(X.view(X.shape[0], -1), blk.mean, blk.has_miss)
        self.comm.allreduce(ssq0)
        blk.rowcnt, blk.ssq0 = rowcnt, float(ssq0.item())

    def _ssq_uncentred(self, blk: BlockState, X: torch.Tensor) -> bool:
        be = self.be
        I = X.shape[0]
        z = lambda n: be.zeros(n, 1)
        out = be.recon_r2(X.view(I, -1), z(I), z(blk.A), z(blk.B), blk.mean) if hasattr(be, "recon_r2") else None
        if out is None:
            return False
        blk.ssq0 = float(self.comm.allreduce(out)[1].item())
        return True

    def _offset_ratio(self, blocks: List[BlockState], Xs: List[torch.Tensor]) -> float:
        worst = 0.0
        for blk, X in zip(blocks, Xs):
            I = X.shape[0]
            sample = X.view(I, -1)[:: max(1, I // 256)][:256].to(torch.float64) - blk.mean
            stat = torch.stack([(sample * sample).sum(), torch.tensor(float(sample.numel()), dtype=torch.float64, device=sample.device)])
            self.comm.allreduce(stat)
            spread = math.sqrt(float(stat[0].item()) / max(float(stat[1].item()), 1.0))
            top = float(blk.mean.abs().max().item())
            if top == 0.0:
                continue
            ratio = top / spread if spread > 0.0 else float("inf")
            worst = ratio if not ratio <= worst else worst
        return worst

    def _probe_plain(self, Xs: List[torch.Tensor], limit: float = 100.0) -> bool:
        flag = torch.zeros(2, dtype=torch.float64, device=Xs[0].device)
        for X in Xs:
            I = X.shape[0]
            sample = X.view(I, -1)[:: max(1, I // 256)][:256].to(torch.float64)
            m = sample.mean(dim=0)
            d = sample - m
            spread = torch.sqrt((d * d).mean())
            bad = (~torch.isfinite(sample)).any().to(torch.float64)
            ratio = torch.where(spread > 0, m.abs().max() / spread, torch.zeros_like(spread))
            flag += torch.stack([bad, (torch.nan_to_num(ratio, nan=float("inf"), posinf=float("inf")) > limit).to(torch.float64)])
        self.comm.allreduce(flag)
        return not bool((flag > 0).any().item())

    def _rank1(self, blk: BlockState, Z: torch.Tensor, wA: torch.Tensor, wB: torch.Tensor,
               info: Optional[torch.Tensor] = None, n_squarings: Optional[int] = None,
               fac: Optional[torch.Tensor] = None, tol: float = 1e-8) -> None:
        order = len(blk.shape)
        if order == 2:
            wB.copy_(Z)
            self.be.normalize(wB)
        elif order == 3:
            self.be.rank1(Z, blk.A, blk.B, wA, wB, info=info, n_squarings=n_squarings)
        else:
            if order > MAX_ORDER:
                raise NotImplementedError(f"X blocks of order > {MAX_ORDER} are not supported")
            dims = blk.shape[1:]
            self.be.rank1_tensor(Z, dims, tol, fac, info=info, n_squarings=None)
            wA.copy_(fac[0, : dims[0]])
            self.kron_trailing([fac[m, : dims[m]] for m in range(1, len(dims))], wB)

    def kron_trailing(self, vecs: List[torch.Tensor], out: torch.Tensor) -> torch.Tensor:
        if len(vecs) == 1:
            out.copy_(vecs[0])
            return out
        acc = vecs[0].contiguous()
        for v in vecs[1:-1]:
            acc = self.be.kron(acc, v.contiguous(), self.be.empty(acc.numel() * v.numel()))
        return self.be.kron(acc, vecs[-1].contiguous(), out)

    def begin(self, Xs: List[torch.Tensor], Y: torch.Tensor, n_components: int, coupled: bool,
              algorithm: str = "direct", owned: Optional[List[bool]] = None, allow_raw: bool = True) -> "FitRun":
        with self.device_ctx():
            return FitRun(self, Xs, Y, n_components, coupled, algorithm, owned, allow_raw)

    def fit(self, Xs: List[torch.Tensor], Y: torch.Tensor, n_components: int, tol: float, max_iter: int,
            coupled: bool, verbose: int = 0, algorithm: str = "direct", use_graphs: bool = False,
            mixed: bool = False, on_preprocessed=None, owned: Optional[List[bool]] = None) -> FitState:
        with self.device_ctx():
            small = self._fit_small(Xs, Y, n_components, tol, max_iter, coupled, verbose, on_preprocessed)
            if small is not None:
                return small
            run = self.begin(Xs, Y, n_components, coupled, algorithm, owned, allow_raw=not mixed)
            if on_preprocessed is not None:
                on_preprocessed(run.blocks)
            run.tol = tol
            run.use_graphs = bool(use_graphs) and getattr(self.be, "name", "") == "hip"
            run.mixed = bool(mixed)
            for a in range(n_components):
                run.start_component(a)
                run.inner_loop(a, max_iter, tol, verbose)
                run.finish_component(a)
            return run.result()

    def _fit_small(self, Xs, Y, n_components, tol, max_iter, coupled, verbose, on_preprocessed) -> Optional[FitState]:
        be = self.be
        if not (self.opt.small_fit and hasattr(be, "fit_small")) or len(Xs) != 1 or self.comm.sharded or verbose:
            return None
        X = Xs[0]
        if X.dtype != torch.float64 or X.dim() not in (2, 3) or X.numel() > self.opt.small_fit_elements or X.shape[0] < 2:
            return None
        validate_limits([tuple(X.shape)], n_components)
        I = X.shape[0]
        A, B = split_trailing(X.shape)
        out = be.fit_small(X.view(I, -1), Y, A, B, n_components, tol, max_iter)
        if out is None:
            return None
        R = n_components
        ssq = out["ssq"]
        loadings = [out["WB"]] if X.dim() == 2 else [out["WA"], out["WB"]]
        blk = BlockState(shape=tuple(X.shape), A=A, B=B, mean=out["x_mean"], has_miss=False, colcnt=None, rowcnt=None,
                         ssq0=float(ssq[0, 0]), dtype=X.dtype, loadings=loadings, r2x=1.0 - ssq[1:, 0] / ssq[0, 0])
        if on_preprocessed is not None:
            on_preprocessed([blk])
        report = {"form": "small_fit", "algorithm": "direct", "launches": 1, "storage": ["float64"], "shapes": [tuple(X.shape)],
                  "missing": [False], "sharded": False, "graphs": False,
                  "note": "the whole fit in one launch of one workgroup (cmtfpls_fit_small_f64); `algorithm` and `graphs` do not apply"}
        return FitState(coupled=coupled, n_components=R, blocks=[blk], T=out["T"], U=out["U"], Q=out["Q"], coef=out["coef"],
                        r2y=1.0 - ssq[1:, 1] / ssq[0, 1], y_mean=out["y_mean"], n_iter=out["n_iter"], n_samples_total=I, report=report)
```

### cmtf_pls_amd/fitrun.py

```python
from __future__ import annotations

import math
from typing import Dict, List, Optional

import numpy as np
import torch

from .fitrun_xcov import XcovMixin
from .state import BlockState, FitState, split_trailing, validate_limits


class FitRun(XcovMixin):

    def __init__(self, eng: NipalsEngine, Xs: List[torch.Tensor], Y: torch.Tensor, n_components: int, coupled: bool,
                 algorithm: str = "direct", owned: Optional[List[bool]] = None, allow_raw: bool = True):
        be, comm = eng.be, eng.comm
        Xs = list(Xs)
        owned = [True] * len(Xs) if owned is None else list(owned)
        if algorithm not in ("direct", "xcov"):
            raise ValueError("algorithm must be 'direct' or 'xcov'")
        self.algorithm_requested = self.algorithm = algorithm
        self.notes: List[str] = []
        validate_limits([tuple(X.shape) for X in Xs], n_components)
        self.eng, self.Xs, self.Y, self.R, self.coupled = eng, Xs, Y, n_components, coupled
        R = n_components
        I, M = Y.shape
        self.I, self.M = I, M
        n_tot = torch.tensor([float(I)], dtype=torch.float64, device=Y.device)
        comm.allreduce(n_tot)
        self.n_total = int(round(float(n_tot.item())))
        want_raw = (allow_raw and algorithm == "xcov" and eng.opt.xcov_raw and eng.opt.xcov_nowrite
                    and n_components <= 64
                    and all(hasattr(be, f) for f in ("axpy_scalar", "total", "recon_r2", "s_downdate", "deflate_contract_yq", "kr_axpy")))
        if not want_raw:
            for b in range(len(Xs)):
                if not owned[b]:
                    Xs[b] = Xs[b].clone()
        ysum, ycnt = be.colstats(Y)
        comm.allreduce(ysum)
        comm.allreduce(ycnt)
        self.y_mean = ysum / ycnt
        _, ssqy0 = be.center(Y, self.y_mean, False)
        comm.allreduce(ssqy0)
        self.ssqy0 = float(ssqy0.item())
        self._ssq_with_s = (want_raw and hasattr(be, "xcov_ssq") and eng.opt.xcov_ssq_with_s)
        self._ssq0_dev = {}
        self._s_prebuilt = {}
        self.blocks = None
        self._stats_with_s = False
        if (want_raw and self._ssq_with_s and eng.opt.xcov_stats_with_s and hasattr(be, "xcov_stats") and M <= 64
                and eng._probe_plain(Xs)):
            self.blocks = self._blocks_from_one_read(Xs)
            self._stats_with_s = self.blocks is not None
            if self.blocks is None:
                self._s_prebuilt, self._ssq0_dev = {}, {}
                self.notes.append("column statistics from the read that builds S declined: a column sum came out non-finite")
        if self.blocks is None:
            self.blocks = [eng._prepare_block(X, self.n_total, defer_centring=want_raw) for X in Xs]
        self.raw = want_raw and not any(blk.has_miss for blk in self.blocks)
        if self.raw:
            ratio = eng._offset_ratio(self.blocks, Xs)
            if not ratio <= eng.opt.xcov_raw_max_offset:
                self.raw = False
                self.notes.append(f"uncentred xcov form declined: max|column mean| / spread = {ratio:.3g} > {eng.opt.xcov_raw_max_offset:g}")
        if self.raw and not self._ssq_with_s:
            self.raw = all(eng._ssq_uncentred(blk, X) for blk, X in zip(self.blocks, Xs))
        if want_raw and not self.raw:
            for b, blk in enumerate(self.blocks):
                if not owned[b]:
                    Xs[b] = Xs[b].clone()
                eng._centre_block(blk, Xs[b])
        if want_raw and not self.raw:
            self._s_prebuilt, self._ssq0_dev, self._stats_with_s = {}, {}, False
        self.X2 = [X.view(I, -1) for X in Xs]
        self.T = be.zeros(I, R)
        self.U = be.zeros(I, R)
        self.Q = be.zeros(M, R)
        self.coef = np.zeros((R, R))
        self.coef_dev = be.zeros(R, R)
        self.b_dev = be.empty(R)
        self.ssq_log = be.zeros(R, len(self.blocks) + 1)
        self.r2y = np.zeros(R)
        for blk in self.blocks:
            blk.loadings = [be.zeros(d, R) for d in blk.shape[1:]]
            blk.r2x = np.zeros(R)
        self.wA = [be.empty(blk.A) for blk in self.blocks]
        for b, blk in enumerate(self.blocks):
            if len(blk.shape) == 2:
                self.wA[b].fill_(1.0)
        self.wB = [be.empty(blk.B) for blk in self.blocks]
        self.Zs = [be.empty(blk.A * blk.B) for blk in self.blocks]
        self.fac = [be.zeros(len(blk.shape) - 1, max(blk.shape[1:])) if len(blk.shape) > 3 else None for blk in self.blocks]
        self.tol = 1e-8
        self.Ts = be.empty(len(self.blocks), I)
        self.t = self.Ts[0] if (len(self.blocks) == 1 and not coupled) else be.empty(I)
        self.status = be.zeros(1 + 2 * len(self.blocks))
        self.status[1::2] = 1.0
        self.status_host = None
        if self.status.is_cuda:
            self.status_host = torch.empty(self.status.shape, dtype=torch.float64, pin_memory=True)
        self.sq_max = int(getattr(be, "rank1_squarings", 30))
        self.sq_budget = [self.sq_max] * len(self.blocks)
        side = int(getattr(be, "rank1_chain_side", 0))
        self.sq_spare = [3 if (len(blk.shape) == 3 and min(blk.A, blk.B) <= side) else 1 for blk in self.blocks]
        self.u = be.empty(I)
        self.u_new = be.empty(I)
        self.q = be.empty(M)
        self.n_iter: List[int] = []
        self.pipeline_stats = {"iterations": 0, "ahead": 0, "unused": 0, "waited": 0, "redone": 0}
        self._executed = 0
        self._parity = 0
        self.mixed = False
        self.use_graphs = False
        self._graphs = {}
        self._graph_error = None
        self._collectives_captured = None
        self._z_ready = False
        self._fused = (algorithm == "direct" and M <= 64
                       and all(hasattr(be, f) for f in ("mode0_contract_yq", "score_gram", "q_update")))
        if self._fused:
            self.Gy = be.empty(M, M)
            self.qbuf = [be.zeros(M), be.zeros(M)]
            self.qpart = be.empty(len(self.blocks), int(be.n_partials) * M)
        elif algorithm == "direct" and comm.sharded:
            self.Gy = be.empty(M, M)
            self.q_prev = be.zeros(M)
        if algorithm == "xcov":
            nb = len(self.blocks)
            self._s_pair = 2 * M <= 64 and eng.opt.xcov_pair_build
            self.S, self.S2, self.S12 = [], [], []
            for blk in self.blocks:
                if blk.has_miss and self._s_pair:
                    both = be.empty(2 * M, blk.A * blk.B)
                    self.S12.append(both)
                    self.S.append(both[:M])
                    self.S2.append(both[M:])
                else:
                    self.S12.append(None)
                    pre = self._s_prebuilt.get(len(self.S))
                    self.S.append(pre if pre is not None else be.empty(M, blk.A * blk.B))
                    self.S2.append(be.empty(M, blk.A * blk.B) if blk.has_miss else None)
            self.rowscale = [(float(blk.A * blk.B) / blk.rowcnt) if blk.has_miss else None for blk in self.blocks]
            any_miss = any(blk.has_miss for blk in self.blocks)
            self.Yw = be.empty(I, 2 * M if self._s_pair else M) if any_miss else None
            self.Gy = be.empty(M, M)
            self.Tq = be.empty(nb, M)
            self.qx = [be.zeros(M), be.zeros(M)]
            self.qc = self.qx[0]
            self.qn = self.Tq[0] if (nb == 1 and not coupled) else be.empty(M)
            self._s_carry = (not any(blk.has_miss for blk in self.blocks)
                             and all(hasattr(be, f) for f in ("s_downdate", "deflate_contract_yq")))
            self._s_ready = False
            self._nowrite = False
            if self.raw:
                self.zM = be.zeros(M)
                self.zA = [be.zeros(blk.A) for blk in self.blocks]
                self.zB = [be.zeros(blk.B) for blk in self.blocks]
            if self._s_carry:
                self.yhat = be.empty(I, 1)
                self.one = be.empty(1)
                self.one.fill_(1.0)
                self.vs = [be.empty(blk.A * blk.B) for blk in self.blocks]
                self._nowrite = eng.opt.xcov_nowrite and hasattr(be, "kr_axpy") and R <= 64
                if self._nowrite:
                    self.dot_log = be.zeros(R, 1 + len(self.blocks))
                    self.Gw = be.empty(R * R)
                    self._G_last = None
                    self._one_read = R > 1 and eng.opt.xcov_one_read and hasattr(be, "score_contract")
                    if self._one_read:
                        self._fused_b = max(range(len(self.blocks)), key=lambda b: self.blocks[b].A * self.blocks[b].B)
                        P0 = self.blocks[self._fused_b].A * self.blocks[self._fused_b].B
                        self.ps = be.empty(P0)
                        self.Rm = be.zeros(P0, R)
                        self.corr = be.empty(I)
                        self.csum = be.empty(1)
            assert self._nowrite or not self.raw, "an uncentred X needs the form of the loop that never writes it"

    def _blocks_from_one_read(self, Xs: List[torch.Tensor]) -> Optional[List[BlockState]]:
        be, comm = self.eng.be, self.eng.comm
        blocks, n = [], float(self.n_total)
        for b, X in enumerate(Xs):
            I = X.shape[0]
            X2 = X.view(I, -1)
            P = X2.shape[1]
            out = be.xcov_stats(X2, self.Y, out=be.empty(self.M, P))
            if out is None:
                return None
            S, stats = out
            comm.allreduce(stats)
            colsum, colsq = stats[:P], stats[P:]
            ssq = (colsq - colsum * colsum / n).sum().reshape(1)
            if not bool(torch.isfinite(ssq).all().item()):
                return None
            A, B = split_trailing(X.shape)
            blocks.append(BlockState(shape=tuple(X.shape), A=A, B=B, mean=colsum / n, has_miss=False, colcnt=None, rowcnt=None,
                                     ssq0=float("nan"), dtype=X.dtype))
            self._s_prebuilt[b] = S
            self._ssq0_dev[b] = ssq
        return blocks

    def start_component(self, a: int) -> None:
        self._executed = 0
        be, comm = self.eng.be, self.eng.comm
        if self.algorithm == "direct":
            self.u.copy_(self.Y[:, 0])
            self._parity = 0
            if self._fused:
                self.qbuf[0].zero_()
                self.qbuf[0][0] = 1.0
            if self._fused or comm.sharded:
                be.gram_tn(self.Y, self.Y, out=self.Gy)
                comm.allreduce(self.Gy)
            return
        for b, blk in enumerate(self.blocks):
            if self._s_ready:
                break
            if self.S12[b] is not None:
                self.Yw[:, :self.M].copy_(self.Y)
                torch.mul(self.Y, self.rowscale[b][:, None], out=self.Yw[:, self.M:])
                be.xcov(self.X2[b], self.Yw, True, out=self.S12[b], mixed=self.mixed)
                comm.allreduce(self.S12[b])
                continue
            if b in self._s_prebuilt:
                del self._s_prebuilt[b]
            elif self.raw and self._ssq_with_s and b not in self._ssq0_dev:
                _, ssq = be.xcov_ssq(self.X2[b], self.Y, blk.mean, out=self.S[b])
                self._ssq0_dev[b] = comm.allreduce(ssq)
            else:
                be.xcov(self.X2[b], self.Y, blk.has_miss, out=self.S[b], mixed=self.mixed)
            comm.allreduce(self.S[b])
            if self.raw:
                ysum, _ = be.colstats(self.Y)
                comm.allreduce(ysum)
                be.s_downdate(self.S[b], blk.A, blk.B, self.zM, self.zA[b], self.zB[b], ysum, blk.mean)
            if blk.has_miss:
                torch.mul(self.Y, self.rowscale[b][:, None], out=self.Yw)
                be.xcov(self.X2[b], self.Yw, True, out=self.S2[b], mixed=self.mixed)
                comm.allreduce(self.S2[b])
        self._s_ready = False
        be.gram_tn(self.Y, self.Y, out=self.Gy)
        comm.allreduce(self.Gy)
        self._parity = 0
        self.qc = self.qx[0]
        self.qc.zero_()
        self.qc[0] = 1.0

    def inner_loop(self, a: int, max_iter: int, tol: float, verbose: int = 0) -> None:
        if max_iter > 0 and self._pipeline_ok():
            self._pipelined = True
            self._inner_loop_xcov_pipelined(a, max_iter, tol, verbose)
            return
        for it in range(max_iter):
            du = self.iterate(it)
            if du is not None and du < tol:
                if verbose:
                    print("Comp {}: converged after {} iterations".format(a, it))
                break

    def _update_budgets(self, host) -> bool:
        retry = False
        for b in range(len(self.blocks)):
            conv, used = host[1 + 2 * b] > 0.5, int(host[2 + 2 * b])
            if used < 0:
                self._chain_gave_up()
                retry = True
                continue
            if not conv and self.sq_budget[b] < self.sq_max:
                self.sq_budget[b] = self.sq_max
                retry = True
            elif conv and len(self.blocks[b].shape) == 3:
                if not self.use_graphs or used + 1 > self.sq_budget[b] or used + 3 < self.sq_budget[b]:
                    self.sq_budget[b] = min(self.sq_max, used + (1 if self.use_graphs else self.sq_spare[b]))
        return retry

    def _peer_failed(self, host, first_attempt: bool) -> bool:
        if not self.eng.comm.sharded:
            return False
        if first_attempt:
            self._nan_tails = 0
        if np.isfinite(float(host[0])) or self._nan_tails > int(getattr(self.eng.comm, "world", 1)):
            return False
        self._nan_tails += 1
        return True

    def _chain_gave_up(self) -> None:
        be = self.eng.be
        if hasattr(be, "rank1_chain_gave_up"):
            be.rank1_chain_gave_up()
        self._graphs.clear()
        self.sq_spare = [1] * len(self.blocks)
        note = "rank-1 chain of squarings in one launch switched off: a workgroup never became resident (GPU shared with another process)"
        if note not in self.notes:
            self.notes.append(note)

    def _read_status(self) -> np.ndarray:
        if self.status_host is None:
            return self.status.cpu().numpy()
        self.status_host.copy_(self.status, non_blocking=True)
        torch.cuda.current_stream(self.status.device).synchronize()
        return self.status_host.numpy()

    def _run(self, key, fn) -> None:
        if not self.use_graphs:
            fn()
            return
        g = self._graphs.get(key)
        if g is not None:
            g.replay()
            return
        fn()
        try:
            g = torch.cuda.CUDAGraph()
            with torch.cuda.graph(g, capture_error_mode="thread_local"):
                fn()
            self._graphs[key] = g
        except Exception as e:
            self.use_graphs = False
            self._graph_error = repr(e)
            self._after_failed_capture()

    def _run_with_collectives(self, key, fn) -> bool:
        if not (self.use_graphs and self.eng.opt.capture_collectives and self._collectives_captured is not False):
            return False
        if not getattr(self.eng.comm, "capturable", False):
            self._collectives_captured = False
            self.notes.append(f"all-reduces not captured into the iteration's graph: the {getattr(self.eng.comm, 'backend', None)} "
                              "backend stages through the host (only RCCL collectives are stream-ordered kernels)")
            return False
        g = self._graphs.get(key)
        if g is not None:
            g.replay()
            return True
        fn()
        try:
            torch.cuda.current_stream().synchronize()
            g = torch.cuda.CUDAGraph()
            with torch.cuda.graph(g, capture_error_mode="thread_local"):
                fn()
            self._graphs[key] = g
            self._collectives_captured = True
        except Exception as e:
            self._collectives_captured = False
            self.notes.append("all-reduces not captured into the iteration's graph: " + repr(e)[:200])
            self._after_failed_capture()
        return True

    def _after_failed_capture(self) -> None:
        try:
            torch.cuda.synchronize()
        except Exception:
            pass
        if hasattr(self.eng.be, "clear_error"):
            self.eng.be.clear_error()

    def iterate(self, it: int) -> Optional[float]:
        if self.algorithm == "xcov":
            return self._iterate_xcov(it)
        be, comm = self.eng.be, self.eng.comm
        if self._fused:
            return self._iterate_fused(it)
        self._executed += 1
        sharded = comm.sharded
        par = self._parity
        u, u_new = (self.u, self.u_new) if par == 0 else (self.u_new, self.u)

        def seg_contract():
            for b, blk in enumerate(self.blocks):
                be.mode0_contract(self.X2[b], u, blk.has_miss, out=self.Zs[b])

        def seg_colscale():
            for b, blk in enumerate(self.blocks):
                if blk.has_miss:
                    be.colscale(self.Zs[b], blk.colcnt, self.n_total)

        def seg_loadings_scores():
            for b, blk in enumerate(self.blocks):
                self.eng._rank1(blk, self.Zs[b], self.wA[b], self.wB[b], info=self.status[1 + 2 * b: 3 + 2 * b],
                                n_squarings=self.sq_budget[b], fac=self.fac[b], tol=self.tol)
                be.score(self.X2[b], blk.A, blk.B, self.wA[b], self.wB[b],
                         blk.rowcnt if blk.has_miss else None, self.Ts[b])
            if self.t.data_ptr() != self.Ts.data_ptr():
                be.scores_mean(self.Ts, self.t)
            be.gram_tn(self.Y, self.t, out=self.q)

        def seg_y_update():
            be.normalize(self.q)
            if sharded:
                be.rowdot(self.Y, self.q, u_new, None)
                be.quadform(self.Gy, self.q, self.q_prev if it > 0 else self.q, self.status[0:1])
            else:
                be.rowdot(self.Y, self.q, u_new, u if it > 0 else None, du2=self.status[0:1])

        first = True
        while True:
            budgets = tuple(self.sq_budget)
            if not sharded:
                def whole():
                    if first:
                        seg_contract()
                        seg_colscale()
                    seg_loadings_scores()
                    seg_y_update()
                self._run(("iter", it > 0, par, budgets, first), whole)
            else:
                if first:
                    self._run(("contract", par), seg_contract)
                    for b in range(len(self.blocks)):
                        comm.allreduce(self.Zs[b])
                    seg_colscale()
                self._run(("loadings", budgets), seg_loadings_scores)
                comm.allreduce(self.q)
                self._run(("yupdate", it > 0, par), seg_y_update)
            host = self._read_status()
            local, peer = self._update_budgets(host), self._peer_failed(host, first)
            if not (local or peer):
                break
            first = False
        if sharded:
            self.q_prev.copy_(self.q)
        self._parity ^= 1
        return None if it == 0 else math.sqrt(max(float(host[0]), 0.0))

    def _iterate_fused(self, it: int) -> Optional[float]:
        be, comm = self.eng.be, self.eng.comm
        self._executed += 1
        sharded = comm.sharded
        par = self._parity
        q_cur, q_new = self.qbuf[par], self.qbuf[par ^ 1]
        nparts = len(self.blocks) * int(be.n_partials)

        def seg_contract():
            for b, blk in enumerate(self.blocks):
                if be.mode0_contract_yq(self.X2[b], self.Y, q_cur, blk.has_miss, out=self.Zs[b]) is None:
                    be.rowdot(self.Y, q_cur, self.u, None)
                    be.mode0_contract(self.X2[b], self.u, blk.has_miss, out=self.Zs[b])

        def seg_colscale():
            for b, blk in enumerate(self.blocks):
                if blk.has_miss:
                    be.colscale(self.Zs[b], blk.colcnt, self.n_total)

        def seg_loadings_scores():
            for b, blk in enumerate(self.blocks):
                self.eng._rank1(blk, self.Zs[b], self.wA[b], self.wB[b], info=self.status[1 + 2 * b: 3 + 2 * b],
                                n_squarings=self.sq_budget[b], fac=self.fac[b], tol=self.tol)
                if be.score_gram(self.X2[b], blk.A, blk.B, self.wA[b], self.wB[b], blk.rowcnt if blk.has_miss else None,
                                 self.Ts[b], self.Y, self.qpart[b]) is None:
                    raise RuntimeError("score_gram refused a shape the fused iteration was planned for")
            if sharded:
                be.q_update(q_new, self.qpart, normalize=False, nparts=nparts)

        def seg_y_update():
            if sharded:
                be.q_update(q_new, None, normalize=True, G=self.Gy, q_prev=q_cur, du2=self.status[0:1])
            else:
                be.q_update(q_new, self.qpart, normalize=True, G=self.Gy, q_prev=q_cur, du2=self.status[0:1], nparts=nparts)

        have_z = self._z_ready and it == 0
        self._z_ready = False
        first = True
        while True:
            budgets = tuple(self.sq_budget)
            if not sharded:
                def whole():
                    if first:
                        if not have_z:
                            seg_contract()
                        seg_colscale()
                    seg_loadings_scores()
                    seg_y_update()
                self._run(("fiter", par, budgets, first, have_z), whole)
            else:
                def whole_sharded():
                    if first:
                        if not have_z:
                            seg_contract()
                        for b in range(len(self.blocks)):
                            comm.allreduce(self.Zs[b])
                        seg_colscale()
                    seg_loadings_scores()
                    comm.allreduce(q_new)
                    seg_y_update()
                if not self._run_with_collectives(("fiter+ar", par, budgets, first, have_z), whole_sharded):
                    if first:
                        if not have_z:
                            self._run(("fcontract", par), seg_contract)
                        for b in range(len(self.blocks)):
                            comm.allreduce(self.Zs[b])
                        seg_colscale()
                    self._run(("floadings", par, budgets), seg_loadings_scores)
                    comm.allreduce(q_new)
                    self._run(("fyupdate", par), seg_y_update)
            host = self._read_status()
            local, peer = self._update_budgets(host), self._peer_failed(host, first)
            if not (local or peer):
                break
            first = False
        self._parity ^= 1
        self.q = q_new
        return None if it == 0 else math.sqrt(max(float(host[0]), 0.0))

    def finish_component(self, a: int) -> None:
        be, comm = self.eng.be, self.eng.comm
        self.n_iter.append(self._executed)
        ssqs = []
        if self.algorithm == "xcov" and self._s_carry:
            if self._nowrite:
                self._finish_xcov_nowrite(a)
            else:
                self._finish_xcov_carry(a)
            return
        if (self.algorithm == "xcov" and len(self.blocks) == 1 and self.blocks[0].has_miss and self.S12[0] is not None
                and a + 1 < self.R and hasattr(be, "xcov_deflate") and self.eng.opt.xcov_deflate_build
                and getattr(self, "_deflate_build_ok", True)):
            if self._finish_xcov_masked_fused(a):
                return
        if self.algorithm == "xcov":
            self.q = self.qc
            if len(self.blocks) == 1:
                blk = self.blocks[0]
                rc = blk.rowcnt if blk.has_miss else None
                s0 = be.score_deflate(self.X2[0], blk.A, blk.B, self.wA[0], self.wB[0], rc, self.t)
                if s0 is None:
                    be.score(self.X2[0], blk.A, blk.B, self.wA[0], self.wB[0], rc, self.t)
                    s0 = be.deflate(self.X2[0], blk.A, blk.B, self.t, self.wA[0], self.wB[0])
                ssqs.append(s0)
            else:
                for b, blk in enumerate(self.blocks):
                    be.score(self.X2[b], blk.A, blk.B, self.wA[b], self.wB[b], blk.rowcnt if blk.has_miss else None, self.Ts[b])
                be.scores_mean(self.Ts, self.t)
                for b, blk in enumerate(self.blocks):
                    ssqs.append(be.deflate(self.X2[b], blk.A, blk.B, self.t, self.wA[b], self.wB[b]))
            be.rowdot(self.Y, self.q, self.u, None)
        if self.algorithm == "direct" and self._fused:
            be.rowdot(self.Y, self.q, self.u, None)
            if self.t.data_ptr() != self.Ts.data_ptr():
                be.scores_mean(self.Ts, self.t)
        elif self.algorithm == "direct" and self._parity == 1:
            self.u.copy_(self.u_new)
            self._parity = 0
        self.T[:, a].copy_(self.t)
        self.U[:, a].copy_(self.u)
        self.Q[:, a].copy_(self.q)
        for b, blk in enumerate(self.blocks):
            if len(blk.shape) == 2:
                blk.loadings[0][:, a].copy_(self.wB[b])
            elif len(blk.shape) == 3:
                blk.loadings[0][:, a].copy_(self.wA[b])
                blk.loadings[1][:, a].copy_(self.wB[b])
            else:
                for m, d in enumerate(blk.shape[1:]):
                    blk.loadings[m][:, a].copy_(self.fac[b][m, :d])
            if self.algorithm == "direct" and not self._fused:
                ssqs.append(be.deflate(self.X2[b], blk.A, blk.B, self.t, self.wA[b], self.wB[b]))
        if self.algorithm == "direct" and self._fused:
            self._finish_fused(a)
            return
        b_dev, _ = self._inner_regression(a)
        for b in range(len(self.blocks)):
            self.ssq_log[a, b].copy_(ssqs[b].reshape(()))
        ssqy = be.y_deflate(self.Y, self.T, a + 1, b_dev, self.q)
        self.ssq_log[a, len(self.blocks)].copy_(ssqy.reshape(()))

    def _inner_regression(self, a: int, extra: Optional[torch.Tensor] = None):
        be, comm = self.eng.be, self.eng.comm
        k = a + 1
        Ta = self.T[:, :k]
        G = be.gram_tn(Ta, Ta)
        g = be.gram_tn(Ta, self.u)
        if comm.sharded:
            packed = torch.cat([G.reshape(-1), g.reshape(-1)] + ([extra.reshape(-1)] if extra is not None else []))
            comm.allreduce(packed)
            G, g = packed[: k * k].view(k, k), packed[k * k: k * k + k]
            extra = packed[k * k + k:] if extra is not None else None
        b_dev = be.normal_solve(G, g.reshape(-1), out=self.b_dev[:k])
        self.coef_dev[:k, a].copy_(b_dev)
        self._G_last = G
        return b_dev, extra

    def _finish_fused(self, a: int) -> None:
        be, comm = self.eng.be, self.eng.comm
        k = a + 1
        b_dev, _ = self._inner_regression(a)
        ssqy = be.y_deflate(self.Y, self.T, k, b_dev, self.q)
        ssqs = []
        self._z_ready = False
        if k < self.R:
            q0 = self.qbuf[0]
            q0.zero_()
            q0[0] = 1.0
            ready = True
            for b, blk in enumerate(self.blocks):
                s_b = be.deflate_contract_yq(self.X2[b], blk.A, blk.B, self.t, self.wA[b], self.wB[b], self.Y, q0,
                                             blk.has_miss, out=self.Zs[b])
                if s_b is None:
                    s_b = be.deflate(self.X2[b], blk.A, blk.B, self.t, self.wA[b], self.wB[b])
                    ready = False
                ssqs.append(s_b)
            self._z_ready = ready
        else:
            for b, blk in enumerate(self.blocks):
                ssqs.append(be.deflate(self.X2[b], blk.A, blk.B, self.t, self.wA[b], self.wB[b]))
        self._log_ssq(a, ssqs, ssqy)

    def _log_ssq(self, a: int, ssqs, ssqy) -> None:
        for b in range(len(self.blocks)):
            self.ssq_log[a, b].copy_(ssqs[b].reshape(()))
        self.ssq_log[a, len(self.blocks)].copy_(ssqy.reshape(()))

    def _store_component(self, a: int) -> None:
        self.T[:, a].copy_(self.t)
        self.U[:, a].copy_(self.u)
        self.Q[:, a].copy_(self.q)
        self._store_loadings(a)

    def _store_loadings(self, a: int) -> None:
        for b, blk in enumerate(self.blocks):
            if len(blk.shape) == 2:
                blk.loadings[0][:, a].copy_(self.wB[b])
            elif len(blk.shape) == 3:
                blk.loadings[0][:, a].copy_(self.wA[b])
                blk.loadings[1][:, a].copy_(self.wB[b])
            else:
                for m, d in enumerate(blk.shape[1:]):
                    blk.loadings[m][:, a].copy_(self.fac[b][m, :d])

    def result(self) -> FitState:
        if getattr(self, "_state", None) is not None:
            return self._state
        nb = len(self.blocks)
        nowrite = self.algorithm == "xcov" and getattr(self, "_nowrite", False)
        for b, ssq in getattr(self, "_ssq0_dev", {}).items():
            self.blocks[b].ssq0 = float(ssq.item())
        self.eng.comm.allreduce(self.ssq_log)
        parts = [self.coef_dev.reshape(-1), self.ssq_log.reshape(-1)]
        if nowrite:
            self.eng.comm.allreduce(self.dot_log)
            parts.append(self.dot_log.reshape(-1))
        host = torch.cat(parts).cpu().numpy()
        R = self.R
        self.coef[...] = host[: R * R].reshape(R, R)
        ssq = host[R * R: R * R + R * (nb + 1)].reshape(R, nb + 1).copy()
        if nowrite:
            dots = host[R * R + R * (nb + 1):].reshape(R, 1 + nb)
            for b, blk in enumerate(self.blocks):
                run = blk.ssq0
                for a in range(len(self.n_iter)):
                    run = run - 2.0 * dots[a, 1 + b] + dots[a, 0]
                    ssq[a, b] = run
        for a in range(len(self.n_iter)):
            for b, blk in enumerate(self.blocks):
                blk.r2x[a] = 1.0 - ssq[a, b] / blk.ssq0
            self.r2y[a] = 1.0 - ssq[a, nb] / self.ssqy0
        self._state = FitState(coupled=self.coupled, n_components=self.R, blocks=self.blocks, T=self.T, U=self.U, Q=self.Q,
                               coef=self.coef, r2y=self.r2y, y_mean=self.y_mean, n_iter=self.n_iter,
                               n_samples_total=self.n_total, report=self.build_report())
        return self._state

    def build_report(self) -> Dict[str, object]:
        eng, comm, nb = self.eng, self.eng.comm, len(self.blocks)
        rep: Dict[str, object] = {
            "form": "regular", "algorithm_requested": self.algorithm_requested, "algorithm": self.algorithm,
            "shapes": [tuple(b.shape) for b in self.blocks], "storage": [str(b.dtype).replace("torch.", "") for b in self.blocks],
            "missing": [bool(b.has_miss) for b in self.blocks], "responses": self.M,
            "sharded": bool(comm.sharded), "world": int(comm.world),
            "graphs": bool(self.use_graphs and self._graphs), "graph_error": self._graph_error,
            "collectives_in_graph": self._collectives_captured is True,
            "backend": getattr(eng.be, "name", type(eng.be).__name__),
        }
        if self.algorithm == "direct":
            rep["y_side"] = "fused into the sweeps" if self._fused else "separate launches"
            if not self._fused and self.M > 64:
                self.notes.append("Y side not fused into the sweeps: more than 64 responses")
            rep["x_passes_per_iteration"] = "2 reads"
            rep["x_passes_per_component"] = ("1 read + write (deflation fused with the next contraction)" if self._fused
                                             else "1 read + write (deflation)")
            rep["x_copy"] = "centred private copy"
        else:
            nowrite = bool(getattr(self, "_nowrite", False))
            one_read = nowrite and bool(getattr(self, "_one_read", False))
            any_miss = any(b.has_miss for b in self.blocks)
            rep["x_copy"] = "none: the caller's uncentred tensor is read in place" if self.raw else "centred private copy"
            rep["raw"] = bool(self.raw)
            rep["x_written"] = not nowrite
            rep["s_carried"] = bool(self._s_carry)
            rep["s_build"] = ("per component (missing values)" if any_miss else "first component only") + \
                             (f", {(self.M + 63) // 64} response tiles of <= 64" if self.M > 64 else "") + \
                             (", [Y, Y * rowscale] in one pass" if any(x is not None for x in self.S12) else "")
            rep["one_read"] = one_read
            rep["stats_with_s"] = bool(getattr(self, "_stats_with_s", False))
            if nowrite:
                rep["x_passes_per_component"] = ("1 read (largest block); 2 reads (other blocks)" if one_read and nb > 1 else
                                                 "1 read" if one_read else "2 reads")
            elif any_miss and nb == 1 and getattr(self, "_deflate_build_ok", True) and self.S12[0] is not None and eng.opt.xcov_deflate_build:
                rep["x_passes_per_component"] = "1 read + 1 read + write (deflation inside the rebuild of S)"
            elif any_miss:
                rep["x_passes_per_component"] = "1 read + write (score + deflation) + S rebuild reads"
            else:
                rep["x_passes_per_component"] = "1 read + 1 read + write"
            rep["pipelined"] = bool(getattr(self, "_pipelined", False))
            if rep["pipelined"]:
                rep["pipeline"] = dict(self.pipeline_stats)
            if not rep["pipelined"] and eng.opt.xcov_pipeline:
                why = ("graph replay requested" if self.use_graphs else "more than 64 responses" if self.M > 64 else
                       "a block of order > 3 or a backend without the single-call iteration")
                self.notes.append("inner loop on S not pipelined: " + why)
            if self.algorithm_requested == "xcov" and not self.raw and eng.opt.xcov_raw and not any_miss and not any("uncentred" in n for n in self.notes):
                self.notes.append("uncentred xcov form declined: " + ("more than 64 components" if self.R > 64 else
                                                                      "f32 matrix precision or a backend without its kernels"))
            if nowrite and eng.opt.xcov_one_read and self.R > 1 and not one_read:
                self.notes.append("one read per component declined: the row does not fit the registers of 1..16 workgroups "
                                  "(rows of 2048..131072 f32 -- 262144 when the last mode divides 4096 -- / 1024..131072 f64 elements, "
                                  "last mode a multiple of 4 / 2)")
        rep["rank1_one_launch_chain"] = bool(getattr(eng.be, "rank1_chain_side", 0)) and any(
            len(blk.shape) == 3 and min(blk.A, blk.B) <= int(getattr(eng.be, "rank1_chain_side", 0)) for blk in self.blocks)
        rep["declined"] = list(self.notes)
        return rep
```

### cmtf_pls_amd/options.py

```python
from __future__ import annotations

from dataclasses import dataclass, replace
from typing import Optional


@dataclass(frozen=True)
class EngineOptions:
    small_fit: bool = True
    small_fit_elements: int = 1 << 15
    xcov_nowrite: bool = True
    xcov_raw: bool = True
    xcov_raw_max_offset: float = 1e4
    xcov_one_read: bool = True
    xcov_pair_build: bool = True
    xcov_ssq_with_s: bool = True
    xcov_stats_with_s: bool = True
    xcov_deflate_build: bool = True
    xcov_pipeline: bool = True
    capture_collectives: bool = False
    project_split_rows: bool = True

    def but(self, **changes) -> "EngineOptions":
        return replace(self, **changes)


_DEFAULT_OPTIONS = EngineOptions()


def default_options() -> EngineOptions:
    return _DEFAULT_OPTIONS


def set_default_options(options: Optional[EngineOptions]) -> EngineOptions:
    global _DEFAULT_OPTIONS
    old, _DEFAULT_OPTIONS = _DEFAULT_OPTIONS, (options if options is not None else EngineOptions())
    return old
```

### include/cmtfpls.h

```cpp
#ifndef CMTFPLS_H
#define CMTFPLS_H

#include <stddef.h>
#include <stdint.h>

#ifdef __cplusplus
extern "C" {
#endif

#define CMTFPLS_OK 0
#define CMTFPLS_EINVAL 1
#define CMTFPLS_EWORKSPACE 2
#define CMTFPLS_EHIP 3
#define CMTFPLS_EUNSUPPORTED 4

int cmtfpls_abi_version(void);
const char* cmtfpls_last_error(void);
int cmtfpls_clear_error(void);
int cmtfpls_status_to_host(const void* src, void* dst_host, size_t bytes, void* event, void* stream);

size_t cmtfpls_colstats_workspace_bytes(int64_t I, int64_t P);
int cmtfpls_colstats_f32(const float* X, int64_t I, int64_t P, double* colsum, double* colcnt,
                         void* ws, size_t ws_bytes, void* stream);
int cmtfpls_colstats_f64(const double* X, int64_t I, int64_t P, double* colsum, double* colcnt,
                         void* ws, size_t ws_bytes, void* stream);
int cmtfpls_sweep_partials(void);
int cmtfpls_center_f32(float* X, int64_t I, int64_t P, const double* mean, double* rowcnt,
                       double* ssq_part, void* stream);
int cmtfpls_center_f64(double* X, int64_t I, int64_t P, const double* mean, double* rowcnt,
                       double* ssq_part, void* stream);

size_t cmtfpls_mode0_contract_workspace_bytes(int64_t I, int64_t P);
int cmtfpls_mode0_contract_f32(const float* X, int64_t I, int64_t P, const double* u, double* Z,
                               int masked, void* ws, size_t ws_bytes, void* stream);
int cmtfpls_mode0_contract_f64(const double* X, int64_t I, int64_t P, const double* u, double* Z,
                               int masked, void* ws, size_t ws_bytes, void* stream);
int cmtfpls_mode0_contract_yq_f32(const float* X, int64_t I, int64_t P, const double* Y, int ldy, int M,
                                  const double* q, double* Z, int masked, void* ws, size_t ws_bytes, void* stream);
int cmtfpls_mode0_contract_yq_f64(const double* X, int64_t I, int64_t P, const double* Y, int ldy, int M,
                                  const double* q, double* Z, int masked, void* ws, size_t ws_bytes, void* stream);
int cmtfpls_colscale_f64(double* Z, int64_t P, const double* colcnt, double n_samples, void* stream);

size_t cmtfpls_rank1_workspace_bytes(int A, int B);
int cmtfpls_rank1_f64(const double* Z, int A, int B, double* wA, double* wB, double* sigma, double* info,
                      int n_squarings, void* ws, size_t ws_bytes, void* stream);
int cmtfpls_rank1_launches_f64(const double* Z, int A, int B, double* wA, double* wB, double* sigma, double* info,
                               int n_squarings, void* ws, size_t ws_bytes, void* stream);
void cmtfpls_rank1_chain_enable(int on);
int cmtfpls_rank1_chain_enabled(void);
int cmtfpls_rank1_score_f64(const double* Z, int A, int B, double* wA, double* wB, double* info, int n_squarings,
                            const double* S, int M, double* tq, void* ws, size_t ws_bytes, void* stream);
int cmtfpls_normalize_f64(double* v, int64_t n, double* nrm, void* stream);
size_t cmtfpls_rank1_tensor_workspace_bytes(const int* dims, int n);
int cmtfpls_rank1_tensor_f64(const double* Z, const int* dims, int n, double tol, double* factors, int ld,
                             double* info, int n_squarings, void* ws, size_t ws_bytes, void* stream);
int cmtfpls_kron_f64(const double* a, int na, const double* b, int nb, double* out, void* stream);

size_t cmtfpls_xcov_workspace_bytes(int64_t I, int64_t P, int M);
int cmtfpls_xcov_f32(const float* X, int64_t I, int64_t P, const double* Y, int ldy, int M, double* S,
                     int masked, void* ws, size_t ws_bytes, void* stream);
int cmtfpls_xcov_f64(const double* X, int64_t I, int64_t P, const double* Y, int ldy, int M, double* S,
                     int masked, void* ws, size_t ws_bytes, void* stream);
int cmtfpls_quadform_f64(const double* G, int M, const double* q, const double* q_old, double* out, void* stream);
int cmtfpls_xcov_deflate_f32(float* X, int64_t I, int A, int B, const double* Y, int ldy, int M, const double* t, const double* wA,
                             const double* wB, double* S, double* ssq, void* ws, size_t ws_bytes, void* stream);
int cmtfpls_xcov_deflate_f64(double* X, int64_t I, int A, int B, const double* Y, int ldy, int M, const double* t, const double* wA,
                             const double* wB, double* S, double* ssq, void* ws, size_t ws_bytes, void* stream);
size_t cmtfpls_xcov_ssq_workspace_bytes(int64_t I, int64_t P, int M);
size_t cmtfpls_xcov_stats_workspace_bytes(int64_t I, int64_t P, int M);
int cmtfpls_xcov_stats_f32(const float* X, int64_t I, int64_t P, const double* Y, int ldy, int M, double* S, double* stats,
                           void* ws, size_t ws_bytes, void* stream);
int cmtfpls_xcov_stats_f64(const double* X, int64_t I, int64_t P, const double* Y, int ldy, int M, double* S, double* stats,
                           void* ws, size_t ws_bytes, void* stream);
int cmtfpls_xcov_ssq_f32(const float* X, int64_t I, int64_t P, const double* Y, int ldy, int M, double* S, const double* mean,
                         double* ssq, void* ws, size_t ws_bytes, void* stream);
int cmtfpls_xcov_ssq_f64(const double* X, int64_t I, int64_t P, const double* Y, int ldy, int M, double* S, const double* mean,
                         double* ssq, void* ws, size_t ws_bytes, void* stream);
int cmtfpls_xcov_iterate_f64(const double* S, int M, int A, int B, const double* q_cur, double* Z, double* wA,
                             double* wB, double* info, int n_squarings, double* q_new, const double* G, double* du2,
                             int first, void* ws_contract, size_t ws_contract_bytes, void* ws_rank1,
                             size_t ws_rank1_bytes, void* stream);
typedef struct {
  const double* S;
  const double* S2;
  const double* colcnt;
  double n_samples;
  int order;
  int A, B;
  int n_squarings;
  double* Z;
  double* wA;
  double* wB;
  double* info;
} cmtfpls_xcov_block;
int cmtfpls_xcov_iterate_blocks_f64(const cmtfpls_xcov_block* blocks, int nb, int M, const double* q_cur, double* tq, double* q_new,
                                    const double* G, double* du2, int first, void* ws_rank1, size_t ws_rank1_bytes, void* stream);
int cmtfpls_s_downdate_f64(double* S, int M, int A, int B, const double* ya, const double* wA, const double* wB,
                           const double* q, const double* v, void* stream);
int cmtfpls_kr_axpy_f64(double* v, int A, int B, const double* WA, const double* WB, int ld, int k, const double* coef, void* stream);
int cmtfpls_axpy_scalar_f64(double* y, int64_t n, const double* a, const double* x, void* stream);
size_t cmtfpls_score_contract_workspace_bytes(int64_t I, int64_t P);
int cmtfpls_score_contract_f32(const float* X, int64_t I, int A, int B, const double* wA, const double* wB, const double* shift,
                               const double* sub_own, const double* add_other, double alpha, double* t, double* Z, double* csum,
                               void* ws, size_t ws_bytes, void* stream);
int cmtfpls_score_contract_f64(const double* X, int64_t I, int A, int B, const double* wA, const double* wB, const double* shift,
                               const double* sub_own, const double* add_other, double alpha, double* t, double* Z, double* csum,
                               void* ws, size_t ws_bytes, void* stream);
int cmtfpls_xcov_f32_mixed(const float* X, int64_t I, int64_t P, const double* Y, int ldy, int M, double* S,
                           int masked, void* ws, size_t ws_bytes, void* stream);
int cmtfpls_mttkrp_f32_mixed(const float* X, int64_t I, int A, int B, const double* WA, const double* WB, int R,
                             double* out, int ldo, void* stream);

int cmtfpls_mttkrp_f32(const float* X, int64_t I, int A, int B, const double* WA, const double* WB, int R,
                       double* out, int ldo, void* stream);
int cmtfpls_mttkrp_f64(const double* X, int64_t I, int A, int B, const double* WA, const double* WB, int R,
                       double* out, int ldo, void* stream);

int cmtfpls_score_f32(const float* X, int64_t I, int A, int B, const double* wA, const double* wB,
                      const double* rowcnt, double* t, void* stream);
int cmtfpls_score_f64(const double* X, int64_t I, int A, int B, const double* wA, const double* wB,
                      const double* rowcnt, double* t, void* stream);
int cmtfpls_score_s_f64(const double* S, int M, int A, int B, const double* wA, const double* wB, double* tq, void* stream);

size_t cmtfpls_deflate_contract_workspace_bytes(int64_t I, int64_t P);
int cmtfpls_deflate_contract_yq_f32(float* X, int64_t I, int A, int B, const double* t, const double* wA,
                                    const double* wB, const double* Y, int ldy, int M, const double* q, double* Z,
                                    int masked, double* ssq, void* ws, size_t ws_bytes, void* stream);
int cmtfpls_deflate_contract_yq_f64(double* X, int64_t I, int A, int B, const double* t, const double* wA,
                                    const double* wB, const double* Y, int ldy, int M, const double* q, double* Z,
                                    int masked, double* ssq, void* ws, size_t ws_bytes, void* stream);
int cmtfpls_score_gram_f32(const float* X, int64_t I, int A, int B, const double* wA, const double* wB,
                           const double* rowcnt, double* t, const double* Y, int ldy, int M, double* qpart,
                           void* stream);
int cmtfpls_score_gram_f64(const double* X, int64_t I, int A, int B, const double* wA, const double* wB,
                           const double* rowcnt, double* t, const double* Y, int ldy, int M, double* qpart,
                           void* stream);
int cmtfpls_q_update_f64(const double* qpart, int nblk, int M, double* q, int normalize, const double* G,
                         const double* q_prev, double* du2, void* stream);

int cmtfpls_deflate_f32(float* X, int64_t I, int A, int B, const double* t, const double* wA,
                        const double* wB, double* ssq_part, void* stream);
int cmtfpls_deflate_f64(double* X, int64_t I, int A, int B, const double* t, const double* wA,
                        const double* wB, double* ssq_part, void* stream);

int cmtfpls_score_deflate_f32(float* X, int64_t I, int A, int B, const double* wA, const double* wB,
                              const double* rowcnt, double* t, double* ssq_part, void* stream);
int cmtfpls_score_deflate_f64(double* X, int64_t I, int A, int B, const double* wA, const double* wB,
                              const double* rowcnt, double* t, double* ssq_part, void* stream);

size_t cmtfpls_small_workspace_bytes(void);
int cmtfpls_gram_tn_f64(const double* A, int lda, int a, const double* B, int ldb, int b, int64_t I,
                        double* C, void* ws, size_t ws_bytes, void* stream);
int cmtfpls_rowdot_f64(const double* Y, int ldy, int M, int64_t I, const double* q, double* u,
                       const double* u_old, double* du2, void* ws, size_t ws_bytes, void* stream);
int cmtfpls_scores_mean_f64(const double* Ts, int nb, int64_t I, double* out, void* stream);
int cmtfpls_y_deflate_f64(double* Y, int ldy, int M, int64_t I, const double* T, int ldt, int R,
                          const double* b, const double* q, double* ssq, void* ws, size_t ws_bytes,
                          void* stream);
int cmtfpls_sum_f64(const double* in, int64_t n, double* out, void* stream);

int cmtfpls_project_rows_f32(const float* X, int64_t I, int A, int B, int R, const double* WA, const double* WB,
                             const double* mean, double* scores, int ld, void* stream);
int cmtfpls_project_rows_f64(const double* X, int64_t I, int A, int B, int R, const double* WA, const double* WB,
                             const double* mean, double* scores, int ld, void* stream);
int cmtfpls_project_rows2_f32(const float* X0, int A0, int B0, const double* WA0, const double* WB0, const double* mean0,
                              const float* X1, int A1, int B1, const double* WA1, const double* WB1, const double* mean1,
                              int64_t I, int R, double* scores, int ld, void* stream);
int cmtfpls_project_rows2_f64(const double* X0, int A0, int B0, const double* WA0, const double* WB0, const double* mean0,
                              const double* X1, int A1, int B1, const double* WA1, const double* WB1, const double* mean1,
                              int64_t I, int R, double* scores, int ld, void* stream);
int cmtfpls_project_rows_idx_f32(const float* X, const int64_t* rows, int64_t n_rows, int A, int B, int R, const double* WA,
                                 const double* WB, const double* mean, double* scores, int ld, void* stream);
int cmtfpls_project_rows_idx_f64(const double* X, const int64_t* rows, int64_t n_rows, int A, int B, int R, const double* WA,
                                 const double* WB, const double* mean, double* scores, int ld, void* stream);
int cmtfpls_project_rows2_idx_f32(const float* X0, int A0, int B0, const double* WA0, const double* WB0, const double* mean0,
                                  const float* X1, int A1, int B1, const double* WA1, const double* WB1, const double* mean1,
                                  const int64_t* rows, int64_t n_rows, int R, double* scores, int ld, void* stream);
int cmtfpls_project_rows2_idx_f64(const double* X0, int A0, int B0, const double* WA0, const double* WB0, const double* mean0,
                                  const double* X1, int A1, int B1, const double* WA1, const double* WB1, const double* mean1,
                                  const int64_t* rows, int64_t n_rows, int R, double* scores, int ld, void* stream);

int cmtfpls_allreduce_sum_f64(void* comm, double* buf, size_t count, void* stream);
int cmtfpls_allreduce_sum_f32(void* comm, float* buf, size_t count, void* stream);

int cmtfpls_normal_solve_f64(const double* G, const double* g, int k, double* b, int incb, void* stream);
size_t cmtfpls_normal_solve_workspace_bytes(int k);
int cmtfpls_normal_solve_ws_f64(const double* G, const double* g, int k, double* b, int incb, void* ws, size_t ws_bytes,
                                void* stream);
int cmtfpls_unit_upper_solve_rows_f64(double* M, int64_t I, int ld, int R, const double* U, const double* shift, int* nan_flag,
                                      void* stream);
int cmtfpls_kr_gram_f64(const double* L, int n, int R, double* G, int first, double scale, void* stream);
int cmtfpls_kr_gram_row_f64(const double* L, int n, int R, int a, double* g, int first, void* stream);
int cmtfpls_khatri_rao_f64(const double* Am, int na, const double* Bm, int nb, int R, double* out, void* stream);
int cmtfpls_predict_rows_f64(const double* S, int64_t I, int lds, int R, const double* Bm, int M, const double* mean,
                             double* out, int ldo, void* stream);
int cmtfpls_recon_f32(const double* T, int64_t I, int ldt, int R, const double* WA, const double* WB, int A, int B,
                      const double* mean, float* out, void* stream);
int cmtfpls_recon_f64(const double* T, int64_t I, int ldt, int R, const double* WA, const double* WB, int A, int B,
                      const double* mean, double* out, void* stream);
size_t cmtfpls_recon_r2_workspace_bytes(int64_t I, int64_t P);
int cmtfpls_recon_r2_f32(const float* X, const double* T, int64_t I, int ldt, int R, const double* WA, const double* WB,
                         int A, int B, const double* mean, double* out, void* ws, size_t ws_bytes, void* stream);
int cmtfpls_recon_r2_f64(const double* X, const double* T, int64_t I, int ldt, int R, const double* WA, const double* WB,
                         int A, int B, const double* mean, double* out, void* ws, size_t ws_bytes, void* stream);

size_t cmtfpls_loo_fold_workspace_bytes(int I, int A, int B, int M, int R);
int cmtfpls_loo_tpls_f64(const double* X, const double* Y, const double* colsum_x, const double* colsum_y, int I, int A,
                         int B, int M, int R, double tol, int max_iter, int fold0, int nfolds, double* Ypred,
                         int* n_iter, void* ws, size_t ws_bytes, void* stream);
size_t cmtfpls_loo_xcov_fold_workspace_bytes(int I, int A, int B, int M, int R);
int cmtfpls_loo_xcov_f64(const double* X, const double* Y, const double* colsum_x, const double* colsum_y, int I, int A,
                         int B, int M, int R, double tol, int max_iter, int fold0, int nfolds, double* Ypred,
                         int* n_iter, void* ws, size_t ws_bytes, void* stream);
typedef struct {
  int I, A, B, M, K, R;
  const int* fold_of;
  double* S;
  double* mean;
  double* Yk;
  double* Gy;
  double* WA;
  double* WB;
  double* Q;
  double* Wa;
  double* Wb;
  double* T;
  double* Gt;
  double* coef;
  double* Rm;
  double* tm;
  double* Tout;
  double* vec;
  int* n_iter;
  int* status;
  double* part;
} cmtfpls_kfold_state;
int cmtfpls_kfold_row_tiles(int64_t I);
int cmtfpls_kfold_part_stride(void);
size_t cmtfpls_kfold_xcov_workspace_bytes(int64_t I, int64_t P, int M, int K);
int cmtfpls_kfold_xcov_f32(const float* X, int64_t I, int A, int B, const double* Y, int M, const int* order, const int* fold_off, int K,
                           const double* ydev, double* S, double* mean, double* stats, void* ws, size_t ws_bytes, void* stream);
int cmtfpls_kfold_xcov_f64(const double* X, int64_t I, int A, int B, const double* Y, int M, const int* order, const int* fold_off, int K,
                           const double* ydev, double* S, double* mean, double* stats, void* ws, size_t ws_bytes, void* stream);
size_t cmtfpls_kfold_inner_workspace_bytes(int A, int B, int K);
int cmtfpls_kfold_inner_f64(const cmtfpls_kfold_state* st, int a, double tol, int max_iter, void* ws, size_t ws_bytes, void* stream);
int cmtfpls_kfold_epilogue_f64(const cmtfpls_kfold_state* st, int stage, int a, const double* in, void* stream);
size_t cmtfpls_kfold_inner_coupled_workspace_bytes(const cmtfpls_kfold_state* blocks, int nb);
int cmtfpls_kfold_inner_coupled_f64(const cmtfpls_kfold_state* blocks, int nb, int a, double tol, int max_iter, void* ws, size_t ws_bytes,
                                    void* stream);
int cmtfpls_kfold_combine_scores_f64(const double* sc, int nb, int64_t n, double* out, void* stream);

size_t cmtfpls_kfold_wide_xcov_workspace_bytes(int64_t I, int64_t P, int W, int K);
int cmtfpls_kfold_wide_xcov_f32(const float* X, int64_t I, int A, int B, const double* Y, int W, const int* order, const int* fold_off,
                                int K, const double* ydev, double* S, double* mean, double* stats, void* ws, size_t ws_bytes, void* stream);
int cmtfpls_kfold_wide_xcov_f64(const double* X, int64_t I, int A, int B, const double* Y, int W, const int* order, const int* fold_off,
                                int K, const double* ydev, double* S, double* mean, double* stats, void* ws, size_t ws_bytes, void* stream);
int cmtfpls_kfold_inner_grouped_f64(const cmtfpls_kfold_state* st, const int* model_fold, int groups, int a, double tol, int max_iter,
                                    void* ws, size_t ws_bytes, void* stream);
int cmtfpls_kfold_epilogue_grouped_f64(const cmtfpls_kfold_state* st, const int* model_fold, int groups, int stage, int a, const double* in,
                                       void* stream);

int cmtfpls_kfold_epilogue_splits_f64(const cmtfpls_kfold_state* st, int splits, int stage, int a, const double* in, void* stream);
size_t cmtfpls_fit_small_workspace_bytes(int I, int A, int B, int M);
int cmtfpls_fit_small_f64(const double* X, const double* Y, int I, int A, int B, int M, int R, double tol, int max_iter,
                          double* T, double* U, double* WA, double* WB, double* Q, double* coef, double* ssq, double* x_mean,
                          double* y_mean, int* n_iter, int* flag, void* ws, size_t ws_bytes, void* stream);

int cmtfpls_add_noise_f32(float* X, int64_t n, double sigma, uint64_t seed, uint64_t offset, double nan_fraction,
                          void* stream);
int cmtfpls_add_noise_f64(double* X, int64_t n, double sigma, uint64_t seed, uint64_t offset, double nan_fraction,
                          void* stream);

int cmtfpls_ceiling_max_blocks(void);
int cmtfpls_ceiling_read(const void* buf, size_t bytes, int64_t row_bytes, int map, float* sink, int blocks, void* stream);
int cmtfpls_ceiling_rmw(void* buf, size_t bytes, int64_t row_bytes, int map, int blocks, void* stream);
int cmtfpls_ceiling_copy(const void* src, void* dst, size_t bytes, int64_t row_bytes, int map, int blocks, void* stream);

#ifdef __cplusplus
}
#endif
#endif
```

Measured before the change: 767.8.

## Fuse rank-1 seed, projection and finish into the persistent syrk chain kernel

Moves the rank-1 seed selection, x/y projections and final normalisation/sign step into the tail of the persistent syrk_chain kernel. Workgroups share the work through chain-flagged global stores and spin-wait loads, so the separate seed_xy and final kernels are no longer launched. This is meant to remove per-iteration launch gaps in the NIPALS loop. The change also sizes the chain grid from an occupancy query, and in exchange adds spin-wait risk, more workspace and a flag to fall back to the old separate path.

```diff
diff --git a/cmtf_pls_amd/_lib.py b/cmtf_pls_amd/_lib.py
--- a/cmtf_pls_amd/_lib.py
+++ b/cmtf_pls_amd/_lib.py
@@ -42,6 +42,7 @@
     "cmtfpls_rank1_score_f64": (c_int, [_P, c_int, c_int, _P, _P, _P, c_int, _P, c_int, _P, _P, c_size_t, _P]),
     "cmtfpls_rank1_f64": (c_int, [_P, c_int, c_int, _P, _P, _P, _P, c_int, _P, c_size_t, _P]),
     "cmtfpls_rank1_launches_f64": (c_int, [_P, c_int, c_int, _P, _P, _P, _P, c_int, _P, c_size_t, _P]),
+    "cmtfpls_rank1_ex_f64": (c_int, [_P, c_int, c_int, _P, _P, _P, _P, c_int, c_int, _P, c_size_t, _P]),
     "cmtfpls_rank1_chain_enable": (None, [c_int]),
     "cmtfpls_rank1_chain_enabled": (c_int, []),
     "cmtfpls_normalize_f64": (c_int, [_P, c_int64, _P, _P]),
diff --git a/cmtf_pls_amd/backend.py b/cmtf_pls_amd/backend.py
--- a/cmtf_pls_amd/backend.py
+++ b/cmtf_pls_amd/backend.py
@@ -112,11 +112,20 @@
         _lib.check(self.lib.cmtfpls_colscale_f64(_ptr(Z), Z.numel(), _ptr(colcnt), float(n_samples), self._stream()), "colscale")
 
     def rank1(self, Z: torch.Tensor, A: int, B: int, wA: torch.Tensor, wB: torch.Tensor,
-              info: Optional[torch.Tensor] = None, n_squarings: Optional[int] = None, launches: bool = False) -> None:
+              info: Optional[torch.Tensor] = None, n_squarings: Optional[int] = None, launches: bool = False,
+              fused_finish: bool = True) -> None:
         ws = self._workspace("rank1", self.lib.cmtfpls_rank1_workspace_bytes(A, B))
-        fn = self.lib.cmtfpls_rank1_launches_f64 if launches else self.lib.cmtfpls_rank1_f64
-        _lib.check(fn(_ptr(Z), A, B, _ptr(wA), _ptr(wB), None, _ptr(info), int(n_squarings or self.rank1_squarings),
-                      _ptr(ws), ws.numel(), self._stream()), "rank1")
+        nsq = int(n_squarings or self.rank1_squarings)
+        if launches:
+            rc = self.lib.cmtfpls_rank1_launches_f64(_ptr(Z), A, B, _ptr(wA), _ptr(wB), None, _ptr(info), nsq, _ptr(ws), ws.numel(),
+                                                     self._stream())
+        else:
+            rc = self.lib.cmtfpls_rank1_ex_f64(_ptr(Z), A, B, _ptr(wA), _ptr(wB), None, _ptr(info), nsq, 0 if fused_finish else 1,
+                                               _ptr(ws), ws.numel(), self._stream())
+        _lib.check(rc, "rank1")
+
+    def rank1_finish_fused(self, A: int, B: int) -> bool:
+        return bool(self.rank1_chain_side) and min(A, B) <= self.rank1_chain_side and A + B <= 3584
 
     def rank1_chain_gave_up(self) -> None:
         self.lib.cmtfpls_rank1_chain_enable(0)
diff --git a/cmtf_pls_amd/csrc/rank1.hip b/cmtf_pls_amd/csrc/rank1.hip
--- a/cmtf_pls_amd/csrc/rank1.hip
+++ b/cmtf_pls_amd/csrc/rank1.hip
@@ -173,6 +173,205 @@
   for (int64_t i = (int64_t)blockIdx.x * 256 + threadIdx.x; i < n; i += (int64_t)gridDim.x * 256) p[i] = kChainEmpty;
 }
 
+__global__ __launch_bounds__(256) void transpose_kernel(const double* __restrict__ Z, int A, int B, double* __restrict__ Zt) {
+  const int64_t idx = (int64_t)blockIdx.x * 256 + threadIdx.x;
+  if (idx >= (int64_t)A * B) return;
+  const int b = (int)(idx / A), a = (int)(idx % A);
+  Zt[idx] = Z[(int64_t)a * B + b];
+}
+
+struct PlainLd { __device__ __forceinline__ double operator()(const double* p) const { return *p; } };
+struct PlainSt { __device__ __forceinline__ void operator()(double* p, double v) const { *p = v; } };
+struct ChainSt { __device__ __forceinline__ void operator()(double* p, double v) const { chain_st(p, v); } };
+struct ChainWaitLd {
+  bool& dead;
+  __device__ __forceinline__ double operator()(const double* p) const {
+    for (int spins = 0;;) {
+      const double v = chain_ld(p);
+      if (!chain_empty(v)) return v;
+      if (dead || ++spins > kChainSpin) { dead = true; return __longlong_as_double(0x7FF8000000000000ll); }
+    }
+  }
+};
+
+__device__ __forceinline__ double sum256(double v, double* slot, int tid) {
+  v = wave_sum(v);
+  if ((tid & 63) == 0) slot[tid >> 6] = v;
+  __syncthreads();
+  double s = 0.0;
+  for (int w = 0; w < 4; ++w) s += slot[w];
+  return s;
+}
+
+template <class LD>
+__device__ __forceinline__ void rank1_seed(LD ld, const double* G, int n, int tid, double* seed, double* red, double* bestv, int* besti) {
+  double bv = -1.0;
+  int bi = 0;
+  for (int i = tid; i < n; i += 256) {
+    const double d = ld(G + (int64_t)i * n + i);
+    if (d > bv) { bv = d; bi = i; }
+  }
+#pragma unroll
+  for (int m = 32; m > 0; m >>= 1) {
+    const double ov = __shfl_xor(bv, m, 64);
+    const int oi = __shfl_xor(bi, m, 64);
+    if (ov > bv || (ov == bv && oi < bi)) { bv = ov; bi = oi; }
+  }
+  if ((tid & 63) == 0) { bestv[tid >> 6] = bv; besti[tid >> 6] = bi; }
+  __syncthreads();
+  bv = bestv[0];
+  bi = besti[0];
+  for (int w = 1; w < 4; ++w)
+    if (bestv[w] > bv || (bestv[w] == bv && besti[w] < bi)) { bv = bestv[w]; bi = besti[w]; }
+  double ss = 0.0;
+  for (int i = tid; i < n; i += 256) {
+    const double g = ld(G + (int64_t)bi * n + i);
+    seed[i] = g;
+    ss = fma(g, g, ss);
+  }
+  const double nrm = sqrt(sum256(ss, red, tid));
+  for (int i = tid; i < n; i += 256) seed[i] = seed[i] / nrm;
+  __syncthreads();
+}
+
+template <class LD, class ST>
+__device__ __forceinline__ void rank1_x_rows(LD ld, ST st, const double* G0, int n, const double* seed, int xb, int tid, double* x) {
+  const int j = xb * 4 + (tid >> 6);
+  const int lane = tid & 63;
+  if (j < n) {
+    double s = 0.0;
+    for (int i = lane; i < n; i += 64) s = fma(ld(G0 + (int64_t)j * n + i), seed[i], s);
+    s = wave_sum(s);
+    if (lane == 0) st(x + j, s);
+  }
+}
+
+template <class ST>
+__device__ __forceinline__ void rank1_y_cols(ST st, const double* M, int n, int k, const double* seed, int yb, int tid, double* rsum, double* y) {
+  const int cx = tid & 31, ry = tid >> 5;
+  const int c = yb * 32 + cx;
+  double s = 0.0;
+  if (c < k)
+    for (int j = ry; j < n; j += 8) s = fma(M[(int64_t)j * k + c], seed[j], s);
+  rsum[ry * 33 + cx] = s;
+  __syncthreads();
+  if (ry == 0 && c < k) {
+    double tot = 0.0;
+#pragma unroll
+    for (int g = 0; g < 8; ++g) tot += rsum[g * 33 + cx];
+    st(y + c, tot);
+  }
+}
+
+__global__ __launch_bounds__(256) void rank1_seed_xy_kernel(const double* __restrict__ M, int n, int k,
+                                                           const double* __restrict__ gbase, int64_t gstride,
+                                                           const double* __restrict__ G0,
+                                                           const Rank1Ctl* __restrict__ ctl, int last_buf, int ny_blocks,
+                                                           double* __restrict__ y, double* __restrict__ x) {
+  extern __shared__ double seed[];
+  __shared__ double red[16];
+  __shared__ double rsum[8 * 33];
+  __shared__ double bestv[4];
+  __shared__ int besti[4];
+  const int fb = (ctl->final_buf >= 0) ? ctl->final_buf : last_buf;
+  rank1_seed(PlainLd{}, gbase + (int64_t)fb * gstride, n, (int)threadIdx.x, seed, red, bestv, besti);
+  if ((int)blockIdx.x >= ny_blocks) rank1_x_rows(PlainLd{}, PlainSt{}, G0, n, seed, (int)blockIdx.x - ny_blocks, (int)threadIdx.x, x);
+  else rank1_y_cols(PlainSt{}, M, n, k, seed, (int)blockIdx.x, (int)threadIdx.x, rsum, y);
+}
+
+__device__ __forceinline__ void rank1_write_info_gv(double* __restrict__ info, const Rank1Ctl* __restrict__ ctl, bool gv) {
+  if (!info) return;
+  if (gv) { info[0] = 0.0; info[1] = -1.0; return; }
+  info[0] = (ctl->done || ctl->last_step >= 0) ? 1.0 : 0.0;
+  info[1] = (double)ctl->steps_used;
+}
+__device__ __forceinline__ bool rank1_gave_up(const double* gave) { return gave && !chain_empty(chain_ld(gave)); }
+__device__ __forceinline__ void rank1_write_info(double* __restrict__ info, const Rank1Ctl* __restrict__ ctl, const double* gave) {
+  if (info) rank1_write_info_gv(info, ctl, rank1_gave_up(gave));
+}
+
+template <int NV>
+__device__ __forceinline__ void rank1_final_core(const double* x, const double* y, int n, int k, int x_is_A, int tid, bool gv,
+                                                 double* red, double* bestv, int* besti, const Rank1Ctl* __restrict__ ctl,
+                                                 double* __restrict__ wA, double* __restrict__ wB,
+                                                 double* __restrict__ sigma, double* __restrict__ info) {
+  constexpr int NT = 1024 / NV;
+  const int lane = tid & 63;
+#pragma unroll
+  for (int r = 0; r < NV; ++r) {
+    const int vt = tid + NT * r;
+    double sx = 0.0, sy = 0.0;
+    for (int i = vt; i < n; i += 1024) sx = fma(x[i], x[i], sx);
+    for (int i = vt; i < k; i += 1024) sy = fma(y[i], y[i], sy);
+    sx = wave_sum(sx);
+    sy = wave_sum(sy);
+    if (lane == 0) { red[vt >> 6] = sx; red[16 + (vt >> 6)] = sy; }
+  }
+  __syncthreads();
+  double nx = 0.0, ny = 0.0;
+  for (int w = 0; w < 16; ++w) nx += red[w];
+  for (int w = 0; w < 16; ++w) ny += red[16 + w];
+  nx = sqrt(nx);
+  ny = sqrt(ny);
+  const double* vb = x_is_A ? y : x;
+  const int nb = x_is_A ? k : n;
+#pragma unroll
+  for (int r = 0; r < NV; ++r) {
+    const int vt = tid + NT * r;
+    double bv = -1.0;
+    int bi = 0;
+    for (int i = vt; i < nb; i += 1024) {
+      const double d = fabs(vb[i]);
+      if (d > bv) { bv = d; bi = i; }
+    }
+#pragma unroll
+    for (int m = 32; m > 0; m >>= 1) {
+      const double ov = __shfl_xor(bv, m, 64);
+      const int oi = __shfl_xor(bi, m, 64);
+      if (ov > bv || (ov == bv && oi < bi)) { bv = ov; bi = oi; }
+    }
+    if (lane == 0) { bestv[vt >> 6] = bv; besti[vt >> 6] = bi; }
+  }
+  __syncthreads();
+  double bv = bestv[0];
+  int bi = besti[0];
+  for (int w = 1; w < 16; ++w)
+    if (bestv[w] > bv || (bestv[w] == bv && besti[w] < bi)) { bv = bestv[w]; bi = besti[w]; }
+  const double sgn = gv ? __longlong_as_double(0x7FF8000000000000ll) : ((vb[bi] < 0.0) ? -1.0 : 1.0);
+  double* ox = x_is_A ? wA : wB;
+  double* oy = x_is_A ? wB : wA;
+  for (int i = tid; i < n; i += NT) ox[i] = sgn * (x[i] / nx);
+  for (int i = tid; i < k; i += NT) oy[i] = sgn * (y[i] / ny);
+  if (tid == 0) {
+    if (sigma) sigma[0] = nx / ny;
+    rank1_write_info_gv(info, ctl, gv);
+  }
+}
+
+__global__ __launch_bounds__(1024) void rank1_final_kernel(const double* __restrict__ x, const double* __restrict__ y,
+                                                          int n, int k, int x_is_A, const Rank1Ctl* __restrict__ ctl,
+                                                          double* __restrict__ wA, double* __restrict__ wB,
+                                                          double* __restrict__ sigma, double* __restrict__ info, const double* gave) {
+  __shared__ double red[32];
+  __shared__ double bestv[16];
+  __shared__ int besti[16];
+  rank1_final_core<1>(x, y, n, k, x_is_A, (int)threadIdx.x, rank1_gave_up(gave), red, bestv, besti, ctl, wA, wB, sigma, info);
+}
+
+struct ChainTail {
+  double* x;
+  double* y;
+  double* stat;
+  double* wA;
+  double* wB;
+  double* sigma;
+  double* info;
+  int x_is_A;
+};
+constexpr int kChainTailScratch = 576;
+constexpr int kChainPanelDoubles = 2 * kTile * (128 + 2);
+constexpr int kChainTailMaxNK = kChainPanelDoubles - kChainTailScratch;
+
 #ifdef CMTFPLS_CHAIN_PROFILE
 __device__ unsigned long long g_chain_prof[1024];
 #define CHAIN_STAMP(slot) do { if (first_wg && tid == 0 && step < 32) g_chain_prof[step * 8 + (slot)] = __builtin_amdgcn_s_memrealtime(); } while (0)
@@ -184,7 +383,7 @@
 
 __global__ __launch_bounds__(kTile* kTile) void syrk_chain_kernel(const double* __restrict__ M0, int n, int k0,
                                                                  double* gbufs, double* trs, double* fros, double* gave_up,
-                                                                 Rank1Ctl* __restrict__ ctl, int n_squarings) {
+                                                                 Rank1Ctl* __restrict__ ctl, int n_squarings, ChainTail tl) {
   constexpr int KC = 128, KW = 8, LDP = KC + 2;
   __shared__ __attribute__((aligned(16))) double pan[2][kTile][LDP];
   __shared__ double red[2][4][kTile * kTile];
@@ -193,6 +392,7 @@
   __shared__ double cfro[2][4];
   __shared__ double ctr[2][kTile];
   __shared__ int cdead[2];
+  __shared__ int tbesti[4 + 16];
   const int tx = threadIdx.x, ty = threadIdx.y, tid = ty * kTile + tx;
   const int lane = tid & 63, wv = tid >> 6, ri = lane & 15, kq = lane >> 4;
   const int nt = (n + kTile - 1) / kTile, nt2 = nt * nt;
@@ -206,6 +406,7 @@
   if (first_wg && tid == 0) { ctl->done = 0; ctl->final_buf = -1; ctl->steps_used = 0; ctl->last_step = -1; }
   if (tid < 2) cdead[tid] = 0;
   int last_step = -1;
+  int final_step = n_squarings;
   for (int step = 0; step <= n_squarings; ++step) {
     if (last_step >= 0) break;
     const int par = step & 1;
@@ -304,8 +505,8 @@
               if (rank_one_out) { ctl->last_step = step; ctl->final_buf = step; }
             }
           }
-          if (rank_one_in) { input_is_result = true; break; }
-          if (rank_one_out) last_step = step;
+          if (rank_one_in) { input_is_result = true; final_step = step - 1; break; }
+          if (rank_one_out) { last_step = step; final_step = step; }
         }
 #pragma unroll
         for (int s2 = 0; s2 < KW; ++s2) {
@@ -347,136 +548,35 @@
     }
     CHAIN_STAMP(6);
   }
-}
-
-__global__ __launch_bounds__(256) void transpose_kernel(const double* __restrict__ Z, int A, int B, double* __restrict__ Zt) {
-  const int64_t idx = (int64_t)blockIdx.x * 256 + threadIdx.x;
-  if (idx >= (int64_t)A * B) return;
-  const int b = (int)(idx / A), a = (int)(idx % A);
-  Zt[idx] = Z[(int64_t)a * B + b];
-}
-
-__global__ __launch_bounds__(256) void rank1_seed_xy_kernel(const double* __restrict__ M, int n, int k,
-                                                           const double* __restrict__ gbase, int64_t gstride,
-                                                           const double* __restrict__ G0,
-                                                           const Rank1Ctl* __restrict__ ctl, int last_buf, int ny_blocks,
-                                                           double* __restrict__ y, double* __restrict__ x) {
-  extern __shared__ double seed[];
-  __shared__ double red[16];
-  __shared__ double rsum[8][33];
-  __shared__ double bestv[4];
-  __shared__ int besti[4];
-  const int fb = (ctl->final_buf >= 0) ? ctl->final_buf : last_buf;
-  const double* G = gbase + (int64_t)fb * gstride;
-  double bv = -1.0;
-  int bi = 0;
-  for (int i = threadIdx.x; i < n; i += 256) {
-    const double d = G[(int64_t)i * n + i];
-    if (d > bv) { bv = d; bi = i; }
-  }
-#pragma unroll
-  for (int m = 32; m > 0; m >>= 1) {
-    const double ov = __shfl_xor(bv, m, 64);
-    const int oi = __shfl_xor(bi, m, 64);
-    if (ov > bv || (ov == bv && oi < bi)) { bv = ov; bi = oi; }
-  }
-  if ((threadIdx.x & 63) == 0) { bestv[threadIdx.x >> 6] = bv; besti[threadIdx.x >> 6] = bi; }
-  __syncthreads();
-  bv = bestv[0];
-  bi = besti[0];
-  for (int w = 1; w < 4; ++w)
-    if (bestv[w] > bv || (bestv[w] == bv && besti[w] < bi)) { bv = bestv[w]; bi = besti[w]; }
-  double ss = 0.0;
-  for (int i = threadIdx.x; i < n; i += 256) {
-    const double g = G[(int64_t)bi * n + i];
-    seed[i] = g;
-    ss = fma(g, g, ss);
-  }
-  const double nrm = sqrt(block_sum(ss, red));
-  for (int i = threadIdx.x; i < n; i += 256) seed[i] = seed[i] / nrm;
-  __syncthreads();
-  if ((int)blockIdx.x >= ny_blocks) {
-    const int j = ((int)blockIdx.x - ny_blocks) * 4 + (threadIdx.x >> 6);
-    const int lane = threadIdx.x & 63;
-    if (j < n) {
-      double s = 0.0;
-      for (int i = lane; i < n; i += 64) s = fma(G0[(int64_t)j * n + i], seed[i], s);
-      s = wave_sum(s);
-      if (lane == 0) x[j] = s;
-    }
-    return;
-  }
-  const int cx = threadIdx.x & 31, ry = threadIdx.x >> 5;
-  const int c = blockIdx.x * 32 + cx;
-  double s = 0.0;
-  if (c < k)
-    for (int j = ry; j < n; j += 8) s = fma(M[(int64_t)j * k + c], seed[j], s);
-  rsum[ry][cx] = s;
-  __syncthreads();
-  if (ry == 0 && c < k) {
-    double tot = 0.0;
-#pragma unroll
-    for (int g = 0; g < 8; ++g) tot += rsum[g][cx];
-    y[c] = tot;
-  }
-}
-
-__device__ __forceinline__ void rank1_write_info(double* __restrict__ info, const Rank1Ctl* __restrict__ ctl, const double* gave) {
-  if (!info) return;
-  if (gave && !chain_empty(chain_ld(gave))) { info[0] = 0.0; info[1] = -1.0; return; }
-  info[0] = (ctl->done || ctl->last_step >= 0) ? 1.0 : 0.0;
-  info[1] = (double)ctl->steps_used;
-}
-
-__device__ __forceinline__ void rank1_final_body(const double* x, const double* y,
-                                                 int n, int k, int x_is_A, const Rank1Ctl* __restrict__ ctl,
-                                                 double* __restrict__ wA, double* __restrict__ wB,
-                                                 double* __restrict__ sigma, double* __restrict__ info, const double* gave) {
-  __shared__ double red[2][16];
-  __shared__ double bestv[16];
-  __shared__ int besti[16];
-  double sx = 0.0, sy = 0.0;
-  for (int i = threadIdx.x; i < n; i += 1024) sx = fma(x[i], x[i], sx);
-  for (int i = threadIdx.x; i < k; i += 1024) sy = fma(y[i], y[i], sy);
-  const double nx = sqrt(block_sum(sx, red[0]));
-  const double ny = sqrt(block_sum(sy, red[1]));
-  const double* vb = x_is_A ? y : x;
-  const int nb = x_is_A ? k : n;
-  double bv = -1.0;
-  int bi = 0;
-  for (int i = threadIdx.x; i < nb; i += 1024) {
-    const double d = fabs(vb[i]);
-    if (d > bv) { bv = d; bi = i; }
-  }
-#pragma unroll
-  for (int m = 32; m > 0; m >>= 1) {
-    const double ov = __shfl_xor(bv, m, 64);
-    const int oi = __shfl_xor(bi, m, 64);
-    if (ov > bv || (ov == bv && oi < bi)) { bv = ov; bi = oi; }
-  }
-  if ((threadIdx.x & 63) == 0) { bestv[threadIdx.x >> 6] = bv; besti[threadIdx.x >> 6] = bi; }
-  __syncthreads();
-  bv = bestv[0];
-  bi = besti[0];
-  for (int w = 1; w < 16; ++w)
-    if (bestv[w] > bv || (bestv[w] == bv && besti[w] < bi)) { bv = bestv[w]; bi = besti[w]; }
-  const bool gv = gave && !chain_empty(chain_ld(gave));
-  const double sgn = gv ? __longlong_as_double(0x7FF8000000000000ll) : ((vb[bi] < 0.0) ? -1.0 : 1.0);
-  double* ox = x_is_A ? wA : wB;
-  double* oy = x_is_A ? wB : wA;
-  for (int i = threadIdx.x; i < n; i += 1024) ox[i] = sgn * (x[i] / nx);
-  for (int i = threadIdx.x; i < k; i += 1024) oy[i] = sgn * (y[i] / ny);
-  if (threadIdx.x == 0) {
-    if (sigma) sigma[0] = nx / ny;
-    rank1_write_info(info, ctl, gave);
-  }
-}
-
-__global__ __launch_bounds__(1024) void rank1_final_kernel(const double* __restrict__ x, const double* __restrict__ y,
-                                                          int n, int k, int x_is_A, const Rank1Ctl* __restrict__ ctl,
-                                                          double* __restrict__ wA, double* __restrict__ wB,
-                                                          double* __restrict__ sigma, double* __restrict__ info, const double* gave) {
-  rank1_final_body(x, y, n, k, x_is_A, ctl, wA, wB, sigma, info, gave);
+  if (!tl.x) return;
+  __syncthreads();
+  double* scr = &pan[0][0][0];
+  double* seed = scr;
+  double* rsum = scr + 256;
+  double* sred = scr + 520;
+  double* sbest = scr + 524;
+  double* fred = scr + 528;
+  double* fbest = scr + 560;
+  double* xs = scr + kChainTailScratch;
+  double* ys = xs + n;
+  ChainWaitLd wl{dead};
+  rank1_seed(wl, gbufs + (int64_t)final_step * nn, n, tid, seed, sred, sbest, tbesti);
+  const int nyb = (k0 + 31) / 32, nxb = (n + 3) / 4;
+  const int nwg = (int)(gridDim.x * gridDim.y), wid = (int)(blockIdx.y * gridDim.x + blockIdx.x);
+  for (int task = wid; task < nyb + nxb; task += nwg) {
+    if (task < nyb) rank1_y_cols(ChainSt{}, M0, n, k0, seed, task, tid, rsum, tl.y);
+    else rank1_x_rows(wl, ChainSt{}, gbufs, n, seed, task - nyb, tid, tl.x);
+    __syncthreads();
+  }
+  const int wdead = __syncthreads_or(dead ? 1 : 0);
+  if (tid == 0) chain_st(tl.stat + wid, wdead ? 1.0 : 0.0);
+  if (!first_wg) return;
+  for (int i = tid; i < n; i += kTile * kTile) xs[i] = wl(tl.x + i);
+  for (int i = tid; i < k0; i += kTile * kTile) ys[i] = wl(tl.y + i);
+  bool other = false;
+  for (int i = tid; i < nwg; i += kTile * kTile) other = other || wl(tl.stat + i) != 0.0;
+  const bool gv = __syncthreads_or((dead || other || rank1_gave_up(gave_up)) ? 1 : 0) != 0;
+  rank1_final_core<4>(xs, ys, n, k0, tl.x_is_A, tid, gv, fred, fbest, tbesti + 4, ctl, tl.wA, tl.wB, tl.sigma, tl.info);
 }
 
 __global__ __launch_bounds__(1024) void rank1_final_score_kernel(const double* __restrict__ x, const double* __restrict__ y,
@@ -574,9 +674,13 @@
 static int chain_slots() {
   static int slots = 0;
   if (slots == 0) {
-    int dev = 0, cus = 0;
+    int dev = 0, cus = 0, per_cu = 0;
     if (hipGetDevice(&dev) != hipSuccess || hipDeviceGetAttribute(&cus, hipDeviceAttributeMultiprocessorCount, dev) != hipSuccess || cus <= 0) cus = 256;
-    slots = 2 * cus;
+    if (hipOccupancyMaxActiveBlocksPerMultiprocessor(&per_cu, reinterpret_cast<const void*>(syrk_chain_kernel), kTile * kTile, 0) != hipSuccess || per_cu <= 0) {
+      (void)hipGetLastError();
+      per_cu = 1;
+    }
+    slots = per_cu * cus;
   }
   return slots;
 }
@@ -591,17 +695,25 @@
   if (A <= 0 || B <= 0) return 0;
   const size_t n = (size_t)(A < B ? A : B), k = (size_t)(A < B ? B : A);
   const size_t nt = (n + kTile - 1) / kTile;
-  const size_t chain = nt * nt <= 256 ? align_up(((size_t)(kChainMaxSteps + 1) * (n * n + nt + nt * nt) + 1) * sizeof(double), 256) : 0;
+  const size_t chain = nt * nt <= 256 ? align_up(((size_t)(kChainMaxSteps + 1) * (n * n + nt + nt * nt) + 1 + n + k + 256) * sizeof(double), 256) : 0;
   return align_up(rank1_ctl_bytes((int)nt), 256) + 3 * align_up(n * n * sizeof(double), 256) +
          align_up((size_t)A * B * sizeof(double), 256) + align_up(n * sizeof(double), 256) + align_up(k * sizeof(double), 256) + chain;
 }
 
 static int rank1_run(const double* Z, int A, int B, double* wA, double* wB, double* sigma, double* info,
-                     int n_squarings, void* ws, size_t ws_bytes, void* stream, const double* S, int M, double* tq, bool allow_chain = true);
+                     int n_squarings, void* ws, size_t ws_bytes, void* stream, const double* S, int M, double* tq, bool allow_chain = true,
+                     bool fused_finish = true);
 
 int cmtfpls_rank1_f64(const double* Z, int A, int B, double* wA, double* wB, double* sigma, double* info,
                       int n_squarings, void* ws, size_t ws_bytes, void* stream) {
   return rank1_run(Z, A, B, wA, wB, sigma, info, n_squarings, ws, ws_bytes, stream, nullptr, 0, nullptr);
+}
+
+int cmtfpls_rank1_ex_f64(const double* Z, int A, int B, double* wA, double* wB, double* sigma, double* info,
+                         int n_squarings, int flags, void* ws, size_t ws_bytes, void* stream) {
+  if (flags & ~CMTFPLS_RANK1_SEPARATE_FINISH) { set_error("rank1_ex: unknown flags"); return CMTFPLS_EINVAL; }
+  return rank1_run(Z, A, B, wA, wB, sigma, info, n_squarings, ws, ws_bytes, stream, nullptr, 0, nullptr, true,
+                   (flags & CMTFPLS_RANK1_SEPARATE_FINISH) == 0);
 }
 
 #ifdef CMTFPLS_CHAIN_PROFILE
@@ -629,7 +741,8 @@
 }
 
 static int rank1_run(const double* Z, int A, int B, double* wA, double* wB, double* sigma, double* info,
-                     int n_squarings, void* ws, size_t ws_bytes, void* stream, const double* S, int M, double* tq, bool allow_chain) {
+                     int n_squarings, void* ws, size_t ws_bytes, void* stream, const double* S, int M, double* tq, bool allow_chain,
+                     bool fused_finish) {
   if (!Z || !wA || !wB || A <= 0 || B <= 0) { set_error("rank1: bad argument"); return CMTFPLS_EINVAL; }
   const int n = A < B ? A : B, k = A < B ? B : A;
   if (n > kTile * kMaxTiles) { set_error("rank1: min(A, B) > 4096 unsupported"); return CMTFPLS_EUNSUPPORTED; }
@@ -672,10 +785,23 @@
     double* fros = trs + steps * nt;
     double* gave_up = fros + steps * (size_t)nt * nt;
     gave = gave_up;
-    const int64_t words = (int64_t)(steps * (nn + nt + (size_t)nt * nt) + 1);
+    const bool fuse = fused_finish && !S && n + k <= kChainTailMaxNK;
+    ChainTail tl{};
+    if (fuse) {
+      tl.x = gave_up + 1;
+      tl.y = tl.x + n;
+      tl.stat = tl.y + k;
+      tl.wA = wA;
+      tl.wB = wB;
+      tl.sigma = sigma;
+      tl.info = info;
+      tl.x_is_A = (A <= B) ? 1 : 0;
+    }
+    const int64_t words = (int64_t)(steps * (nn + nt + (size_t)nt * nt) + 1) + (fuse ? (int64_t)(n + k + nt * nt) : 0);
     hipLaunchKernelGGL(chain_preset_kernel, dim3((unsigned)((words + 2047) / 2048)), dim3(256), 0, st, reinterpret_cast<unsigned long long*>(chain_region), words);
     const dim3 cgrid(nt, (g_chain_on.load(std::memory_order_relaxed) == 2 && nt > 1) ? nt - 1 : nt);
-    hipLaunchKernelGGL(syrk_chain_kernel, cgrid, block, 0, st, M0, n, k, gbufs, trs, fros, gave_up, ctl, n_squarings);
+    hipLaunchKernelGGL(syrk_chain_kernel, cgrid, block, 0, st, M0, n, k, gbufs, trs, fros, gave_up, ctl, n_squarings, tl);
+    if (fuse) return check_launch("rank1");
     hipLaunchKernelGGL(rank1_seed_xy_kernel, dim3(ny_blocks + (n + 3) / 4), dim3(256), (size_t)n * sizeof(double), st,
                        M0, n, k, gbufs, (int64_t)nn, gbufs, ctl, n_squarings, ny_blocks, yv, xv);
   } else {
diff --git a/cmtf_pls_amd/engine.py b/cmtf_pls_amd/engine.py
--- a/cmtf_pls_amd/engine.py
+++ b/cmtf_pls_amd/engine.py
@@ -124,7 +124,10 @@
             wB.copy_(Z)
             self.be.normalize(wB)
         elif order == 3:
-            self.be.rank1(Z, blk.A, blk.B, wA, wB, info=info, n_squarings=n_squarings)
+            if self.opt.fused_iteration_tail:
+                self.be.rank1(Z, blk.A, blk.B, wA, wB, info=info, n_squarings=n_squarings)
+            else:
+                self.be.rank1(Z, blk.A, blk.B, wA, wB, info=info, n_squarings=n_squarings, fused_finish=False)
         else:
             if order > MAX_ORDER:
                 raise NotImplementedError(f"X blocks of order > {MAX_ORDER} are not supported")
diff --git a/cmtf_pls_amd/fitrun.py b/cmtf_pls_amd/fitrun.py
--- a/cmtf_pls_amd/fitrun.py
+++ b/cmtf_pls_amd/fitrun.py
@@ -672,6 +672,11 @@
             rep["y_side"] = "fused into the sweeps" if self._fused else "separate launches"
             if not self._fused and self.M > 64:
                 self.notes.append("Y side not fused into the sweeps: more than 64 responses")
+            fin = getattr(eng.be, "rank1_finish_fused", None)
+            fused_fin = [bool(eng.opt.fused_iteration_tail and fin is not None and len(b.shape) == 3 and fin(b.A, b.B))
+                         for b in self.blocks]
+            rep["iteration_tail"] = ["rank-1 finish inside the chain launch" if f else "separate rank-1 finish kernels"
+                                     for f in fused_fin]
             rep["x_passes_per_iteration"] = "2 reads"
             rep["x_passes_per_component"] = ("1 read + write (deflation fused with the next contraction)" if self._fused
                                              else "1 read + write (deflation)")
diff --git a/cmtf_pls_amd/options.py b/cmtf_pls_amd/options.py
--- a/cmtf_pls_amd/options.py
+++ b/cmtf_pls_amd/options.py
@@ -19,6 +19,7 @@
     xcov_pipeline: bool = True
     capture_collectives: bool = False
     project_split_rows: bool = True
+    fused_iteration_tail: bool = True
 
     def but(self, **changes) -> "EngineOptions":
         return replace(self, **changes)
diff --git a/include/cmtfpls.h b/include/cmtfpls.h
--- a/include/cmtfpls.h
+++ b/include/cmtfpls.h
@@ -46,6 +46,9 @@
                       int n_squarings, void* ws, size_t ws_bytes, void* stream);
 int cmtfpls_rank1_launches_f64(const double* Z, int A, int B, double* wA, double* wB, double* sigma, double* info,
                                int n_squarings, void* ws, size_t ws_bytes, void* stream);
+#define CMTFPLS_RANK1_SEPARATE_FINISH 1
+int cmtfpls_rank1_ex_f64(const double* Z, int A, int B, double* wA, double* wB, double* sigma, double* info,
+                         int n_squarings, int flags, void* ws, size_t ws_bytes, void* stream);
 void cmtfpls_rank1_chain_enable(int on);
 int cmtfpls_rank1_chain_enabled(void);
 int cmtfpls_rank1_score_f64(const double* Z, int A, int B, double* wA, double* wB, double* info, int n_squarings,
```

Result: no change. 767.0, median of 6 (-0.1%).
